# NVlabs/FasterViT

Measured on AMD Instinct MI355X. Metric: images/sec FasterViT-0 224x224 inference, bs=256/GPU, higher is better.
Workload: dtype f16; 1 GPU; faster_vit_0_224 inference, 224x224, batch 256/GPU, synthetic weights (tests/synth.py init family); global_batch=256, parallelism=dp1 (independent shards, no data-path collective), hat_operands=f16, streams=1

## Files before the change

fastervit_amd/csrc/fvit_api.hip:

```cpp
#include <stdarg.h>
#include <stdlib.h>
#include <string.h>

#include <algorithm>
#include <map>
#include <mutex>
#include <string>
#include <vector>

#include "fvit_common.h"

namespace fvit {

static thread_local char g_err[512] = "";

void set_error(const char* fmt, ...) {
    va_list ap;
    va_start(ap, fmt);
    vsnprintf(g_err, sizeof(g_err), fmt, ap);
    va_end(ap);
}

int check_launch(const char* what) {
    hipError_t e = hipGetLastError();
// ... 120 lines not shown
    L.off_SLAB = L.off_CNT = 0;
    if (d.C == 512 && winmlp_supported(d.C, d.hidden)) {
        L.off_SLAB = take(winmlp_split_slab_bytes(L.Mx, d.C, 4));
        L.off_CNT = take((size_t)(L.Mx / 32 + 8) * 4);
    }
    L.off_SPLITK = 0;
    L.splitk_bytes = 0;
    if (tune_get("gemm_splitk", 0)) {
        const int slots = tune_get("gemm_splitk_slots", 460);
        auto need = [&](int64_t rows) -> size_t {
            if (rows <= 0) return 0;
            const int64_t tiles = ((rows + 127) / 128) * ((d.C + 127) / 128);
            const int64_t sp = std::min<int64_t>(8, slots / std::max<int64_t>(tiles, 1));
            return sp >= 2 ? (size_t)sp * rows * d.C * 4 : 0;
        };
        const size_t nb = std::max(need(L.Mx), d.hier ? need(L.Mc) : (size_t)0);
        if (nb > 0) { L.off_SPLITK = take(nb); L.splitk_bytes = nb; }
    }
    L.total = off;
    const int want_s = fvit_attention_spad(L.S), want_g = d.hier ? fvit_attention_spad(L.G) : d.gpad;
    if (d.spad != want_s || d.gpad != want_g) {
        set_error("stage descriptor: spad/gpad %d/%d do not match fvit_attention_spad (%d/%d)", d.spad, d.gpad, want_s, want_g);
        return false;
    }
    return true;
}

#define FVIT_TRY(expr)            \
    do {                          \
        int rc__ = (expr);        \
        if (rc__ != FVIT_OK) return rc__; \
    } while (0)

static AttnBlkCall attnblk_call(int dtype, const float* srcA, int rowsA, const float* srcB, int rowsB, const int32_t* src_idx,
                                const int32_t* add_idx, const float* add, const float* ln_w, const float* ln_b, float eps, int rows_per_image,
                                const void* w_qkv_frag, const float* b_qkv_heads, const void* w_proj_frag, const float* b_proj,
                                const float* gamma, const float* bias, float* x_out, int nwin, int S, int heads, int C, float scale) {
    return {dtype, srcA, rowsA, srcB, rowsB, src_idx, add_idx, add, ln_w, ln_b, eps, rows_per_image, w_qkv_frag,
            b_qkv_heads, w_proj_frag, b_proj, gamma, bias, x_out, nwin, S, heads, C, scale};
}

static MlpFusedCall mlp_fused_call(int dtype, float* x, int M, int C, int hidden, const float* ln_w, const float* ln_b, float eps,
                                   const void* w_fc1_frag, const float* b_fc1, const void* w_fc2_frag, const float* b_fc2, const float* gamma) {
    return {dtype, x, M, C, hidden, ln_w, ln_b, eps, w_fc1_frag, b_fc1, w_fc2_frag, b_fc2, gamma};
}

static CtBlkCall ctblk_call(int dtype, const float* X, int rowsA, const int32_t* src_idx, const float* add, float* R, int batch, int G,
                            int heads, int C, int hidden, const float* ln1_w, const float* ln1_b, const void* w_qkv_frag,
                            const float* b_qkv_heads, const void* w_proj_frag, const float* b_proj, const float* gamma1, const float* bias,
                            float scale, const float* ln2_w, const float* ln2_b, const void* w_fc1_frag, const float* b_fc1,
                            const void* w_fc2_frag, const float* b_fc2, const float* gamma2, float eps) {
    return {dtype, X, rowsA, src_idx, add, R, batch, G, heads, C, hidden, ln1_w, ln1_b, w_qkv_frag, b_qkv_heads, w_proj_frag,
            b_proj, gamma1, bias, scale, ln2_w, ln2_b, w_fc1_frag, b_fc1, w_fc2_frag, b_fc2, gamma2, eps};
}

enum class CarrierRoute {
    NONE,
    FUSED_CT,
    ATTNBLK,
    LNGEMM_CHAIN,
    CHAIN,
};
enum class WinAttnRoute {
    WINBLK,
    ATTNBLK,
    LNGEMM_PREADDED,
    CHAIN,
};
enum class MlpRoute {
    WINMLP,
    MLP_FUSED,
    LNGEMM_CHAIN,
    CHAIN,
};

struct BlockRoute {
    CarrierRoute carrier = CarrierRoute::NONE;
    MlpRoute carrier_mlp = MlpRoute::CHAIN;
    WinAttnRoute window_attn = WinAttnRoute::CHAIN;
    MlpRoute window_mlp = MlpRoute::CHAIN;
    bool preadd_eligible = false;
    const float* pe_next = nullptr;
    int win_blk_split = 1, win_mlp_split = 1;
};

struct RouteKnobs {
    const int ln_gemm = tune_get("ln_gemm", 0), ln_gemm_max_rows = tune_get("ln_gemm_max_rows", 16384);
    const int attn_fused = tune_get("attn_fused", 1), attn_fused_x2 = tune_get("attn_fused_x2", 1);
    const int attn_fused_min_rows = tune_get("attn_fused_min_rows", 16384), attn_fused512_min_rows = tune_get("attn_fused512_min_rows", 1 << 30);
    const int mlp_fused = tune_get("mlp_fused", 1);
    const int mlp_fused_min_rows = tune_get("mlp_fused_min_rows", 16384), mlp_fused512_min_rows = tune_get("mlp_fused512_min_rows", 1 << 30);
    const int win_mlp = tune_get("win_mlp", 1), win_mlp256 = tune_get("win_mlp256", 2), win_mlp_split = tune_get("win_mlp_split", 1);
    const int win_fused = tune_get("win_fused", 1), win_fused256 = tune_get("win_fused256", 0), win_blk_split = tune_get("win_blk_split", 1);
    const int ct_fused = tune_get("ct_fused", 1), pe_preadd = tune_get("pe_preadd", 1);
};

static BlockRoute choose_route(const FvitStageDesc& d, const StageLayout& L, const FvitBlockWeights& w, const RouteKnobs& k) {
    const int T = d.weight_terms;
    auto ln_gemm_ok = [&](int N, int ldo, int64_t rows) {
        return T == 1 && ln_gemm_supported(d.C, N, L.ldn, ldo) && k.ln_gemm && rows <= k.ln_gemm_max_rows;
    };
    auto attnblk = [&](const FvitAttnWeights& a, int S, int64_t rows) {
        const bool terms_ok = T == 1 || (T == 2 && d.C == 256 && S > 48 && k.attn_fused_x2);
        return terms_ok && a.w_qkv_frag && a.b_qkv_heads && a.w_proj_frag && d.dpad == 32 && d.C / d.heads == 32 && attnblk_supported(d.C, d.heads, S) &&
               rows >= (d.C == 256 ? k.attn_fused_min_rows : k.attn_fused512_min_rows) && k.attn_fused;
    };
    auto mlp = [&](const FvitMlpWeights& m, int64_t rows) {
        const bool frags = m.w_fc1_frag && m.w_fc2_frag;
        if (T <= 2 && frags && winmlp_supported(d.C, d.hidden) && (d.C == 512 ? k.win_mlp != 0 : rows >= k.mlp_fused_min_rows && k.win_mlp256 != 0))
            return MlpRoute::WINMLP;
        if (T == 1 && frags && mlp_fused_supported(d.C, d.hidden) && rows >= (d.C == 256 ? k.mlp_fused_min_rows : k.mlp_fused512_min_rows) && k.mlp_fused)
            return MlpRoute::MLP_FUSED;
        return ln_gemm_ok(d.hidden, L.ldh, rows) ? MlpRoute::LNGEMM_CHAIN : MlpRoute::CHAIN;
    };

    BlockRoute r;
    r.win_blk_split = k.win_blk_split;
    r.win_mlp_split = k.win_mlp_split;
    if (d.hier) {
        const FvitAttnWeights& a = w.hat_attn;
        if (T <= 2 && ctblk_supported(d.C, d.heads, L.G, d.hidden) && d.dpad == 32 && a.w_qkv_frag && a.b_qkv_heads && a.w_proj_frag && a.bias &&
            w.hat_mlp.w_fc1_frag && w.hat_mlp.w_fc2_frag && k.ct_fused)
            r.carrier = CarrierRoute::FUSED_CT;
        else if (attnblk(a, L.G, L.Mc))
            r.carrier = CarrierRoute::ATTNBLK;
        else
            r.carrier = ln_gemm_ok(L.ldqkv, L.ldqkv, L.Mc) ? CarrierRoute::LNGEMM_CHAIN : CarrierRoute::CHAIN;
        r.carrier_mlp = mlp(w.hat_mlp, L.Mc);
    }
    const FvitAttnWeights& a = w.attn;
    if (T <= 2 && (T == 1 || d.C == 512) && winblk_supported(d.C, d.heads, L.S) && d.dpad == 32 && a.w_qkv_frag && a.b_qkv_heads && a.w_proj_frag && a.bias &&
        (d.C == 512 ? k.win_fused != 0 : k.win_fused256 != 0))
        r.window_attn = WinAttnRoute::WINBLK;
    else if (attnblk(a, L.S, L.Mx))
        r.window_attn = WinAttnRoute::ATTNBLK;
    r.window_mlp = mlp(w.mlp, L.Mx);
    r.preadd_eligible = !d.hier && r.window_attn == WinAttnRoute::CHAIN && (r.window_mlp == MlpRoute::CHAIN || r.window_mlp == MlpRoute::LNGEMM_CHAIN) &&
                        ln_gemm_ok(L.ldqkv, L.ldqkv, L.Mx) && k.pe_preadd;
    return r;
}

struct Branch {
    float* x;
    int64_t rows;
    void *xn, *qkv, *ao, *h;
    int nwin, S;
};

static LnCall ln_call(const FvitStageDesc& d, const StageLayout& L, const float* ln_w, const float* ln_b, const float* src, int64_t rows, void* n_out) {
    LnCall ln = {d.operand_dtype, src, 0, nullptr, 0, nullptr, nullptr, nullptr, nullptr, n_out, L.at * L.ldn, ln_w, ln_b, 1e-5f, (int)rows, 1, d.C};
    if (L.at == 2) ln.lo_off = L.ldn;
    return ln;
}

enum class AttnStart { QKV_GEMM, CORE };

static int run_attn(const FvitStageDesc& d, const StageLayout& L, const FvitAttnWeights& w, AttnStart start, const Branch& b, char* ws, hipStream_t st) {
    const int dt = d.operand_dtype;
    const int T = d.weight_terms;
    const int AT = L.at;
    dbg_rowhash("attn.xn", b.xn, b.rows, AT * L.ldn * 2, st);
    if (start == AttnStart::QKV_GEMM) {
        GemmCall g1 = {dt, b.xn, AT * L.ldn, w.w_qkv, T * L.ldn, w.b_qkv, nullptr, b.qkv, AT * L.ldqkv, (int)b.rows, L.ldqkv, T * L.ldn, 0};
        g1.ka = L.ldn;
        if (AT == 2) g1.out_lo_off = L.ldqkv;
        FVIT_TRY(launch_gemm(g1, st));
    }
    dbg_rowhash("attn.qkv", b.qkv, b.rows, AT * L.ldqkv * 2, st);
    AttnCall at = {dt, b.qkv, AT * L.ldqkv, b.ao, AT * L.ldao, w.bias, b.nwin, b.S, d.heads, d.dpad, L.scale, w.rel_table, w.rel_w, w.rel_ng, d.C / d.heads};
    if (AT == 2) { at.q_lo_off = L.ldqkv; at.o_lo_off = L.ldao; }
    FVIT_TRY(launch_attention(at, st));
    dbg_rowhash("attn.ao", b.ao, b.rows, AT * L.ldao * 2, st);
    GemmCall g2 = {dt, b.ao, AT * L.ldao, w.w_proj, T * L.ldao, w.b_proj, w.gamma, b.x, d.C, (int)b.rows, d.C, T * L.ldao, 2};
    g2.ka = L.ldao;
    if (L.splitk_bytes) { g2.splitk_slab = (float*)(ws + L.off_SPLITK); g2.splitk_bytes = L.splitk_bytes; }
    FVIT_TRY(launch_gemm(g2, st));
    dbg_rowhash("attn.out", b.x, b.rows, d.C * 4, st);
    return FVIT_OK;
}

static int run_mlp(const FvitStageDesc& d, const StageLayout& L, const FvitMlpWeights& w, MlpRoute route, const BlockRoute& r, const Branch& b,
                   const FvitStageTables& t, char* ws, hipStream_t st) {
    const int dt = d.operand_dtype;
    const int T = d.weight_terms, AT = L.at;
    switch (route) {
    case MlpRoute::WINMLP: {
        MlpFusedCall mc = mlp_fused_call(dt, b.x, (int)b.rows, d.C, d.hidden, w.ln_w, w.ln_b, 1e-5f, w.w_fc1_frag, w.b_fc1, w.w_fc2_frag, w.b_fc2, w.gamma);
        mc.terms = T;
        if (L.off_SLAB) {
            mc.slab = (float*)(ws + L.off_SLAB);
            mc.counters = (int*)(ws + L.off_CNT);
            mc.nsplit = r.win_mlp_split;
        }
        FVIT_TRY(launch_winmlp(mc, st));
        dbg_rowhash("winmlp.out", b.x, b.rows, d.C * 4, st);
        return FVIT_OK;
    }
    case MlpRoute::MLP_FUSED: {
        MlpFusedCall mc = mlp_fused_call(dt, b.x, (int)b.rows, d.C, d.hidden, w.ln_w, w.ln_b, 1e-5f, w.w_fc1_frag, w.b_fc1, w.w_fc2_frag, w.b_fc2, w.gamma);
        dbg_rowhash("mlpf.in", b.x, b.rows, d.C * 4, st);
        FVIT_TRY(launch_mlp_fused(mc, st));
        dbg_rowhash("mlpf.out", b.x, b.rows, d.C * 4, st);
        return FVIT_OK;
    }
    case MlpRoute::LNGEMM_CHAIN: {
        LnGemmCall lg = {ln_call(d, L, w.ln_w, w.ln_b, b.x, b.rows, b.xn), w.w_fc1, L.ldn, w.b_fc1, b.h, L.ldh, d.hidden, 1};
        FVIT_TRY(launch_ln_gemm(lg, st));
        break;
    }
    case MlpRoute::CHAIN: {
        FVIT_TRY(launch_gather_layernorm(ln_call(d, L, w.ln_w, w.ln_b, b.x, b.rows, b.xn), st));
        GemmCall g1 = {dt, b.xn, AT * L.ldn, w.w_fc1, T * L.ldn, w.b_fc1, nullptr, b.h, AT * L.ldh, (int)b.rows, d.hidden, T * L.ldn, 1};
        g1.ka = L.ldn;
        if (AT == 2) g1.out_lo_off = L.ldh;
        FVIT_TRY(launch_gemm(g1, st));
        break;
    }
    }
    dbg_rowhash("mlp.h", b.h, b.rows, AT * L.ldh * 2, st);
    GemmCall g2 = {dt, b.h, AT * L.ldh, w.w_fc2, T * L.ldh, w.b_fc2, w.gamma, b.x, d.C, (int)b.rows, d.C, T * L.ldh, 2};
    g2.ka = L.ldh;
    if (r.pe_next) { g2.add = r.pe_next; g2.add_idx = t.ln1_add; g2.rows_per_image = L.rpi; }
    if (L.splitk_bytes) { g2.splitk_slab = (float*)(ws + L.off_SPLITK); g2.splitk_bytes = L.splitk_bytes; }
    FVIT_TRY(launch_gemm(g2, st));
    dbg_rowhash("mlp.out", b.x, b.rows, d.C * 4, st);
    return FVIT_OK;
}

static AttnBlkCall window_attnblk_call(const FvitStageDesc& d, const StageLayout& L, const FvitBlockWeights& w, const FvitStageTables& t, float* X, float* R) {
    const FvitAttnWeights& a = w.attn;
    AttnBlkCall ab = attnblk_call(d.operand_dtype, X, L.rpi, R, L.G, (d.hier ? t.ln1_src : nullptr), t.ln1_add, w.pe_x, a.ln_w, a.ln_b, 1e-5f, L.rpi,
                                  a.w_qkv_frag, a.b_qkv_heads, a.w_proj_frag, a.b_proj, a.gamma, a.bias, X, d.batch * L.nW, L.S, d.heads, d.C, L.scale);
    ab.terms = d.weight_terms;
    return ab;
}

static int run_block(const FvitStageDesc& d, const StageLayout& L, const BlockRoute& r, const FvitBlockWeights& w, const FvitStageTables& t,
                     char* ws, hipStream_t st) {
    const int dt = d.operand_dtype;
    float* X = (float*)(ws + L.off_X);
    float* R = (float*)(ws + L.off_R);
    const Branch win = {X, L.Mx, ws + L.off_Xn, ws + L.off_QKV, ws + L.off_AO, ws + L.off_H, d.batch * L.nW, L.S};
    const Branch ct = {R, L.Mc, ws + L.off_Rn, ws + L.off_RQKV, ws + L.off_RAO, ws + L.off_RH, d.batch, L.G};

    const FvitAttnWeights& ha = w.hat_attn;
    const float* pe_ct = d.square ? w.pe_ct : nullptr;
    LnCall ct_ln = ln_call(d, L, ha.ln_w, ha.ln_b, X, L.Mc, ct.xn);
    ct_ln.rowsA = L.rpi; ct_ln.src_idx = t.ct_src; ct_ln.add = pe_ct; ct_ln.x_out = R; ct_ln.rows_per_image = L.G;
    switch (r.carrier) {
    case CarrierRoute::NONE:
        break;
    case CarrierRoute::FUSED_CT: {
        const FvitMlpWeights& hm = w.hat_mlp;
        CtBlkCall cb = ctblk_call(dt, X, L.rpi, t.ct_src, pe_ct, R, d.batch, L.G, d.heads, d.C, d.hidden, ha.ln_w, ha.ln_b, ha.w_qkv_frag,
                                  ha.b_qkv_heads, ha.w_proj_frag, ha.b_proj, ha.gamma, ha.bias, L.scale, hm.ln_w, hm.ln_b, hm.w_fc1_frag, hm.b_fc1,
                                  hm.w_fc2_frag, hm.b_fc2, hm.gamma, 1e-5f);
        cb.terms = d.weight_terms;
        FVIT_TRY(launch_ctblk(cb, st));
        dbg_rowhash("ct.block", R, L.Mc, d.C * 4, st);
        break;
    }
    case CarrierRoute::ATTNBLK: {
        AttnBlkCall ab = attnblk_call(dt, X, L.rpi, nullptr, 0, t.ct_src, nullptr, pe_ct, ha.ln_w, ha.ln_b, 1e-5f, L.G, ha.w_qkv_frag, ha.b_qkv_heads,
                                      ha.w_proj_frag, ha.b_proj, ha.gamma, ha.bias, R, d.batch, L.G, d.heads, d.C, L.scale);
        FVIT_TRY(launch_attnblk(ab, st));
        dbg_rowhash("ct.attnblk", R, L.Mc, d.C * 4, st);
        break;
    }
    case CarrierRoute::LNGEMM_CHAIN: {
        LnGemmCall lg = {ct_ln, ha.w_qkv, L.ldn, ha.b_qkv, ct.qkv, L.ldqkv, L.ldqkv, 0};
        FVIT_TRY(launch_ln_gemm(lg, st));
        FVIT_TRY(run_attn(d, L, ha, AttnStart::CORE, ct, ws, st));
        break;
    }
    case CarrierRoute::CHAIN:
        FVIT_TRY(launch_gather_layernorm(ct_ln, st));
        dbg_rowhash("ct.gather", R, L.Mc, d.C * 4, st);
        FVIT_TRY(run_attn(d, L, ha, AttnStart::QKV_GEMM, ct, ws, st));
        break;
    }
    if (r.carrier != CarrierRoute::NONE && r.carrier != CarrierRoute::FUSED_CT) FVIT_TRY(run_mlp(d, L, w.hat_mlp, r.carrier_mlp, r, ct, t, ws, st));

    const FvitAttnWeights& a = w.attn;
    switch (r.window_attn) {
    case WinAttnRoute::WINBLK: {
        AttnBlkCall ab = window_attnblk_call(d, L, w, t, X, R);
        if (L.off_SLAB) {
            ab.slab = (float*)(ws + L.off_SLAB);
            ab.counters = (int*)(ws + L.off_CNT);
            ab.nsplit = r.win_blk_split;
        }
        FVIT_TRY(launch_winblk(ab, st));
        dbg_rowhash("win.winblk", X, L.Mx, d.C * 4, st);
        break;
    }
    case WinAttnRoute::ATTNBLK:
        FVIT_TRY(launch_attnblk(window_attnblk_call(d, L, w, t, X, R), st));
        dbg_rowhash("win.attnblk", X, L.Mx, d.C * 4, st);
        break;
    case WinAttnRoute::LNGEMM_PREADDED: {
        LnGemmCall lg = {ln_call(d, L, a.ln_w, a.ln_b, X, L.Mx, nullptr), a.w_qkv, L.ldn, a.b_qkv, win.qkv, L.ldqkv, L.ldqkv, 0};
        FVIT_TRY(launch_ln_gemm(lg, st));
        FVIT_TRY(run_attn(d, L, a, AttnStart::CORE, win, ws, st));
        break;
    }
    case WinAttnRoute::CHAIN: {
        LnCall ln1 = ln_call(d, L, a.ln_w, a.ln_b, X, L.Mx, win.xn);
        ln1.rowsA = L.rpi; ln1.srcB = R; ln1.rowsB = L.G; ln1.src_idx = d.hier ? t.ln1_src : nullptr; ln1.add_idx = t.ln1_add; ln1.add = w.pe_x;
        ln1.x_out = X; ln1.rows_per_image = L.rpi;
        FVIT_TRY(launch_gather_layernorm(ln1, st));
        dbg_rowhash("win.gather", X, L.Mx, d.C * 4, st);
        FVIT_TRY(run_attn(d, L, a, AttnStart::QKV_GEMM, win, ws, st));
        break;
    }
    }
    return run_mlp(d, L, w.mlp, r.window_mlp, r, win, t, ws, st);
}

static int check_hat_call(const FvitStageDesc* desc, bool args_ok, const FvitStageTables* t, const void* workspace, size_t workspace_bytes,
                          const void* carrier, const char* no_carrier, StageLayout& L) {
    if (!desc || !args_ok) {
        set_error("null argument");
        return FVIT_EINVAL;
    }
    const FvitStageDesc& d = *desc;
    if (!make_layout(d, L)) return FVIT_EINVAL;
    if (!t || !t->ln1_add || (d.hier && (!t->ln1_src || !t->ct_src)) || (d.hier && d.do_propagation && !t->up_idx)) {
        set_error("stage tables missing (ln1_add%s)", d.hier ? ", ln1_src, ct_src, up_idx" : "");
        return FVIT_EINVAL;
    }
    if (!workspace || workspace_bytes < L.total) {
        set_error("workspace too small: %zu < %zu", workspace_bytes, L.total);
        return FVIT_EWORKSPACE;
    }
    if (d.hier && !carrier) {
        set_error("%s", no_carrier);
        return FVIT_EINVAL;
    }
    return FVIT_OK;
}

}

using namespace fvit;

extern "C" {

int fvit_abi_version(void) { return FVIT_ABI_VERSION; }
const char* fvit_last_error(void) { return g_err; }

int fvit_attention_dense(int32_t S, int32_t dpad) { return attention_dense(S, dpad) ? 1 : 0; }

int fvit_attention_spad(int32_t S) {
    int sb = (S + 15) / 16;
    if (sb == 9) sb = 10;
    if (sb == 11 || sb == 12) sb = 13;
    return sb * 16;
}

size_t fvit_stage_workspace_bytes(const FvitStageDesc* desc) {
    StageLayout L;
    if (!desc || !make_layout(*desc, L)) return 0;
    return L.total;
}

int fvit_workspace_init(const FvitStageDesc* desc, void* workspace, size_t bytes, fvit_stream_t stream) {
    StageLayout L;
    if (!desc || !make_layout(*desc, L)) return FVIT_EINVAL;
    if (!workspace || bytes < L.total) {
        set_error("workspace too small: %zu < %zu", bytes, L.total);
        return FVIT_EWORKSPACE;
    }
    if (hipMemsetAsync(workspace, 0, L.total, (hipStream_t)stream) != hipSuccess) return check_launch("workspace memset");
    return FVIT_OK;
}

int fvit_hat_stage_forward(const FvitStageDesc* desc, const FvitBlockWeights* blocks, const FvitStageTables* tables,
                           const FvitMapView* in, const float* ct_init, const FvitMapView* out, void* workspace,
                           size_t workspace_bytes, fvit_stream_t stream) {
    return fvit_hat_stage_forward_tail(desc, blocks, tables, in, ct_init, out, nullptr, workspace, workspace_bytes, stream);
}

int fvit_rows_avgpool(int32_t round_dtype, const float* x, float* out, int32_t B, int32_t rows, int32_t C, fvit_stream_t stream) {
    return launch_rows_avgpool(x, out, B, rows, C, round_dtype, (hipStream_t)stream);
}

int fvit_hat_stage_forward_tail(const FvitStageDesc* desc, const FvitBlockWeights* blocks, const FvitStageTables* tables,
                                const FvitMapView* in, const float* ct_init, const FvitMapView* out, const FvitStageTail* tail,
                                void* workspace, size_t workspace_bytes, fvit_stream_t stream) {
    StageLayout L;
    const bool pooled = tail && tail->pool_out;
    FVIT_TRY(check_hat_call(desc, blocks && in && (out || pooled), tables, workspace, workspace_bytes, ct_init, "hierarchical stage needs ct_init", L));
    const FvitStageDesc& d = *desc;
    if (tail && (!tail->ln_w != !tail->ln_b || (pooled && tail->ln_w))) {
        set_error("stage tail: LayerNorm2d needs both ln_w and ln_b, and excludes pool_out");
        return FVIT_EINVAL;
    }
    if (pooled && (d.hier || L.nW != 1 || L.ncw != 0 || d.H != d.Hp || d.W != d.Wp)) {
        set_error("stage tail: pool_out needs one window per image and no carrier tokens (hier=%d, %d windows, map %dx%d of %dx%d)", d.hier, L.nW, d.H, d.W,
                  d.Hp, d.Wp);
        return FVIT_EINVAL;
    }
    hipStream_t st = (hipStream_t)stream;
    char* ws = (char*)workspace;
    float* X = (float*)(ws + L.off_X);
    PartitionCall pc = {*in, d.batch, d.C, d.Hp, d.Wp, d.ws, X, L.S, L.ncw, d.hier ? ct_init : nullptr, L.ncw};
    FVIT_TRY(launch_partition(pc, st));
    dbg_rowhash("partition", X, L.Mx, d.C * 4, st);
    const RouteKnobs knobs{};
    std::vector<BlockRoute> routes;
    for (int i = 0; i < d.depth; ++i) routes.push_back(choose_route(d, L, blocks[i], knobs));
    for (int i = 0; i + 1 < d.depth; ++i) {
        if (routes[i].preadd_eligible && routes[i + 1].preadd_eligible && blocks[i + 1].pe_x) {
            routes[i].pe_next = blocks[i + 1].pe_x;
            routes[i + 1].window_attn = WinAttnRoute::LNGEMM_PREADDED;
        }
    }
    for (int i = 0; i < d.depth; ++i) FVIT_TRY(run_block(d, L, routes[i], blocks[i], *tables, ws, st));
    if (pooled)
        return launch_rows_avgpool(X, tail->pool_out, d.batch, L.S, d.C, tail->pool_dtype, st);
    const bool prop = d.hier && d.do_propagation && d.depth > 0 && blocks[d.depth - 1].last;
    ReverseCall rc = {X, L.S, L.ncw, d.batch, d.C, d.Hp, d.Wp, d.H, d.W, d.ws, *out,
                      prop ? blocks[d.depth - 1].hat_attn.gamma : nullptr, prop ? tables->up_idx : nullptr};
    if (tail && tail->ln_w) return launch_reverse_ln(rc, tail->ln_w, tail->ln_b, tail->ln_eps, st);
    FVIT_TRY(launch_reverse(rc, st));
    return FVIT_OK;
}

int fvit_hat_block_forward(const FvitStageDesc* desc, const FvitBlockWeights* block, const FvitStageTables* tables, float* x,
                           float* ct, void* workspace, size_t workspace_bytes, fvit_stream_t stream) {
    StageLayout L;
    FVIT_TRY(check_hat_call(desc, block && x, tables, workspace, workspace_bytes, ct, "hierarchical block needs carrier tokens", L));
    const FvitStageDesc& d = *desc;
    hipStream_t st = (hipStream_t)stream;
    char* ws = (char*)workspace;
    float* X = (float*)(ws + L.off_X);
    const int nwin = d.batch * L.nW;
    FVIT_TRY(launch_ct_copy(X, L.S, L.ncw, L.nloc, x, nwin, d.C, 1, st));
    if (d.hier) FVIT_TRY(launch_ct_copy(X, L.S, 0, L.ncw, ct, nwin, d.C, 1, st));
    FVIT_TRY(run_block(d, L, choose_route(d, L, *block, RouteKnobs{}), *block, *tables, ws, st));
    if (d.hier && block->last && d.do_propagation)
        FVIT_TRY(launch_propagate(X, block->hat_attn.gamma, tables->up_idx, L.S, L.ncw, L.nloc, nwin, d.C, st));
    FVIT_TRY(launch_ct_copy(X, L.S, L.ncw, L.nloc, x, nwin, d.C, 0, st));
    if (d.hier) FVIT_TRY(launch_ct_copy(X, L.S, 0, L.ncw, ct, nwin, d.C, 0, st));
    return FVIT_OK;
}

int fvit_token_init(const FvitMapView* in, const float* weight, const float* bias, float* ct_out, int32_t batch, int32_t C, int32_t Hp,
                    int32_t Wp, int32_t pool_kh, int32_t pool_kw, int32_t pool_sh, int32_t pool_sw, int32_t cw, fvit_stream_t stream) {
    if (!in || !weight || !bias || !ct_out) { set_error("null argument"); return FVIT_EINVAL; }
    return launch_token_init(*in, weight, bias, ct_out, batch, C, Hp, Wp, pool_kh, pool_kw, pool_sh, pool_sw, cw, (hipStream_t)stream);
}

int fvit_window_partition(const FvitMapView* in, int32_t batch, int32_t C, int32_t Hp, int32_t Wp, int32_t ws, float* windows,
                          fvit_stream_t stream) {
    if (!in || !windows) { set_error("null argument"); return FVIT_EINVAL; }
    PartitionCall pc = {*in, batch, C, Hp, Wp, ws, windows, ws * ws, 0, nullptr, 0};
    return launch_partition(pc, (hipStream_t)stream);
}

int fvit_window_reverse(const float* windows, int32_t batch, int32_t C, int32_t Hp, int32_t Wp, int32_t H, int32_t W, int32_t ws,
                        const FvitMapView* out, fvit_stream_t stream) {
    if (!out || !windows) { set_error("null argument"); return FVIT_EINVAL; }
    ReverseCall rc = {windows, ws * ws, 0, batch, C, Hp, Wp, H, W, ws, *out, nullptr, nullptr};
    return launch_reverse(rc, (hipStream_t)stream);
}

int fvit_gemm_bias_act(int32_t operand_dtype, const void* A, int32_t lda, const void* Wt, int32_t ldw, const float* bias, void* out,
                       int32_t ldo, int32_t M, int32_t N, int32_t K, int32_t act, fvit_stream_t stream) {
    GemmCall g = {operand_dtype, A, lda, Wt, ldw, bias, nullptr, out, ldo, M, N, K, act ? 1 : 0};
    return launch_gemm(g, (hipStream_t)stream);
}

int fvit_gemm_residual(int32_t operand_dtype, const void* A, int32_t lda, const void* Wt, int32_t ldw, const float* bias,
                       const float* gamma, float* x, int32_t ldx, int32_t M, int32_t N, int32_t K, fvit_stream_t stream) {
    GemmCall g = {operand_dtype, A, lda, Wt, ldw, bias, gamma, x, ldx, M, N, K, 2};
    return launch_gemm(g, (hipStream_t)stream);
}

int fvit_gemm_residual_splitk(int32_t operand_dtype, const void* A, int32_t lda, const void* Wt, int32_t ldw, const float* bias, const float* gamma,
                              float* x, int32_t ldx, int32_t M, int32_t N, int32_t K, float* slab, size_t slab_bytes, fvit_stream_t stream) {
    GemmCall g = {operand_dtype, A, lda, Wt, ldw, bias, gamma, x, ldx, M, N, K, 2};
    g.splitk_slab = slab;
    g.splitk_bytes = slab_bytes;
    return launch_gemm(g, (hipStream_t)stream);
}

int fvit_gemm_terms(int32_t operand_dtype, const void* A, int32_t lda, const void* Wt, int32_t ldw, const float* bias, const float* gamma,
                    void* out, int32_t ldo, int32_t M, int32_t N, int32_t K, int32_t ka, int32_t epilogue, fvit_stream_t stream) {
    if (epilogue < 0 || epilogue > 2) { set_error("gemm_terms: epilogue %d", epilogue); return FVIT_EINVAL; }
    GemmCall g = {operand_dtype, A, lda, Wt, ldw, bias, epilogue == 2 ? gamma : nullptr, out, ldo, M, N, K, epilogue};
    g.ka = ka;
    return launch_gemm(g, (hipStream_t)stream);
}

int fvit_gemm_terms_lo(int32_t operand_dtype, const void* A, int32_t lda, const void* Wt, int32_t ldw, const float* bias, const float* gamma,
                       void* out, int32_t ldo, int32_t out_lo_off, int32_t M, int32_t N, int32_t K, int32_t ka, int32_t epilogue,
                       fvit_stream_t stream) {
    if (epilogue < 0 || epilogue > 2) { set_error("gemm_terms_lo: epilogue %d", epilogue); return FVIT_EINVAL; }
    GemmCall g = {operand_dtype, A, lda, Wt, ldw, bias, epilogue == 2 ? gamma : nullptr, out, ldo, M, N, K, epilogue};
    g.ka = ka;
    g.out_lo_off = out_lo_off;
    return launch_gemm(g, (hipStream_t)stream);
}

int fvit_window_attention_terms(int32_t operand_dtype, const void* qkv, int32_t ldq, int32_t q_lo_off, void* out, int32_t ldo,
// ... 310 lines not shown
```

fastervit_amd/csrc/fvit_attnblk.hip:

```cpp
#include "fvit_common.h"

namespace fvit {

namespace {

struct AttnBlkParams {
    const float* srcA;
    const float* srcB;
    const int32_t* src_idx;
    const int32_t* add_idx;
    const float* add;
    const float* ln_w;
    const float* ln_b;
    float eps;
    int rowsA, rowsB, rows_per_image;
    const void* wqkv_f;
    const float* bqkv;
    const void* wproj_f;
    const float* bproj;
    const float* gamma;
    const float* bias;
    float* x_out;
    int nwin, S, heads;
    float scale;
    int ablate;
    unsigned long long* ts;
    int stagger;
};

__device__ __forceinline__ void glds16(const void* gsrc, char* lds_dst) {
    __builtin_amdgcn_global_load_lds((const __attribute__((address_space(1))) void*)gsrc,
                                     (__attribute__((address_space(3))) void*)lds_dst, 16, 0, 0);
}

template <typename T, int CC, int NRB, int NW, bool BIAS_LDS, bool DBQ = false, bool TS = false, int WT = 1>
__global__ __launch_bounds__(64 * NW, (CC == 256 && WT == 1) ? 2 : 1) void attnblk_kernel(AttnBlkParams p) {
    static_assert(WT == 1 || (WT == 2 && DBQ && !BIAS_LDS && !TS), "two weight terms: DBQ form, bias from L2");
    typedef typename Op16<T>::v8 v8;
#define FVIT_AB_STAMP(k) if constexpr (TS) { if ((threadIdx.x & 63) == 0) p.ts[((size_t)blockIdx.x * NW + (threadIdx.x >> 6)) * 16 + (k)] = __builtin_amdgcn_s_memtime(); }
    FVIT_AB_STAMP(0)
    typedef typename Op16<T>::v4 v4;
    constexpr int C = CC, KK = C / 32, CB = C / 16;
    constexpr int SP = NRB * 16;
    constexpr int WPW = NW / NRB;
    constexpr int NKB32 = (NRB + 1) / 2;
    constexpr int QKV_FRAGS = 6 * KK;
    constexpr int QKV_BYTES = QKV_FRAGS * 1024, PROJ_BYTES = CB * 1024, BIAS_BYTES = BIAS_LDS ? SP * SP * 4 : 0;
    constexpr int KX_BYTES = NW * 1024;
    constexpr int VX_BYTES = WPW * 2 * NKB32 * 1024;
    constexpr int OFF_PROJ = (DBQ ? 2 : 1) * QKV_BYTES, OFF_BIAS = OFF_PROJ + WT * PROJ_BYTES, OFF_KX = OFF_BIAS + ((BIAS_BYTES + 1023) / 1024) * 1024;
    constexpr int OFF_VX = OFF_KX + KX_BYTES, OFF_BQ = OFF_VX + VX_BYTES;
    constexpr int MAX_HEADS = CC / 32;
    constexpr int OFF_BP = OFF_BQ + MAX_HEADS * 96 * 4;
    __shared__ __attribute__((aligned(16))) char smem[OFF_BP + 2 * CC * 4];

    const int tid = threadIdx.x;
    const int lane = tid & 63;
    const int wave = __builtin_amdgcn_readfirstlane(tid >> 6);
    const int g = lane >> 4, s = lane & 15;
    const int lane16 = lane * 16;
    const int wi = wave / NRB, qb = wave - wi * NRB;
    const int win = blockIdx.x * WPW + wi;
    const bool win_ok = win < p.nwin;
    const int tok = qb * 16 + s;
    const bool row_ok = win_ok && tok < p.S;
    const int64_t row = (int64_t)(win_ok ? win : p.nwin - 1) * p.S + (tok < p.S ? tok : p.S - 1);
    float* bqs = (float*)(smem + OFF_BQ);
    float* bps = (float*)(smem + OFF_BP);
    float* gms = bps + CC;

    const char* __restrict__ Wq = (const char*)p.wqkv_f;
    const char* __restrict__ Wp = (const char*)p.wproj_f;

    auto dma_qkv = [&](int h, int slot, int term = 0) {
        const char* src = Wq + ((size_t)term * p.heads + h) * QKV_BYTES + lane16;
        char* dst = smem + slot * QKV_BYTES;
#pragma unroll
        for (int i = 0; i < QKV_FRAGS / NW; ++i) glds16(src + (wave + NW * i) * 1024, dst + (wave + NW * i) * 1024);
    };
    auto dma_proj_bias = [&](int h) {
        const char* src = Wp + (size_t)h * PROJ_BYTES + lane16;
#pragma unroll
        for (int i = 0; i < CB / NW; ++i) glds16(src + (wave + NW * i) * 1024, smem + OFF_PROJ + (wave + NW * i) * 1024);
        if constexpr (WT == 2) {
            const char* src2 = Wp + ((size_t)p.heads + h) * PROJ_BYTES + lane16;
#pragma unroll
            for (int i = 0; i < CB / NW; ++i) glds16(src2 + (wave + NW * i) * 1024, smem + OFF_PROJ + PROJ_BYTES + (wave + NW * i) * 1024);
        }
        if (BIAS_LDS) {
            const char* bsrc = (const char*)(p.bias + (size_t)h * SP * SP) + lane16;
            constexpr int BP = (BIAS_BYTES + 1023) / 1024;
#pragma unroll
            for (int i = 0; i < (BP + NW - 1) / NW; ++i) {
                const int piece = wave + NW * i;
                if (piece < BP) glds16(bsrc + piece * 1024, smem + OFF_BIAS + piece * 1024);
            }
        }
    };

    for (int i = tid; i < p.heads * 96; i += 64 * NW) bqs[i] = p.bqkv[i];
    for (int i = tid; i < CC; i += 64 * NW) {
        bps[i] = p.bproj[i];
        gms[i] = p.gamma ? p.gamma[i] : 1.0f;
    }
    if (NRB == 1) {
        for (int i = tid; i < VX_BYTES / 4; i += 64 * NW) ((float*)(smem + OFF_VX))[i] = 0.f;
    }
    const int hrot = p.stagger ? (int)((blockIdx.x >> 3) % (unsigned)p.heads) : 0;
    auto head_of = [&](int it) { const int hh = it + hrot; return hh >= p.heads ? hh - p.heads : hh; };
    dma_qkv(head_of(0), 0);
    if constexpr (WT == 2) dma_qkv(head_of(0), 1, 1);

    const float* src;
    const float* addp = nullptr;
    {
        const int b = (int)(row / p.rows_per_image), pr = (int)(row - (int64_t)b * p.rows_per_image);
        if (p.src_idx) {
            const int si = p.src_idx[pr];
            src = si >= 0 ? p.srcA + ((size_t)b * p.rowsA + si) * C : p.srcB + ((size_t)b * p.rowsB + (-si - 1)) * C;
        } else {
            src = p.srcA + (size_t)row * C;
        }
        if (p.add) {
            const int ai = p.add_idx ? p.add_idx[pr] : pr;
            if (ai >= 0) addp = p.add + (size_t)ai * C;
        }
    }
    constexpr bool KEEPX = CC == 256;
    v8 xf[KK];
    f4 v[KK][2];
    {
        float sum = 0.f;
#pragma unroll
        for (int kk = 0; kk < KK; ++kk)
#pragma unroll
            for (int h2 = 0; h2 < 2; ++h2) {
                const int co = (kk >> 1) * 64 + g * 16 + (kk & 1) * 8 + h2 * 4;
                f4 t = *(const f4*)(src + co);
                if (addp) t += *(const f4*)(addp + co);
                v[kk][h2] = t;
                sum += (t[0] + t[1]) + (t[2] + t[3]);
            }
        sum = sum_xor32(sum_xor16(sum));
        if constexpr (TS) { asm volatile("s_nop 0" ::"v"(sum) : "memory"); }
        FVIT_AB_STAMP(1)
        const float mean = sum / (float)C;
        float sq = 0.f;
#pragma unroll
        for (int kk = 0; kk < KK; ++kk)
#pragma unroll
            for (int h2 = 0; h2 < 2; ++h2) {
                const f4 d = v[kk][h2] - mean;
                sq += (d[0] * d[0] + d[1] * d[1]) + (d[2] * d[2] + d[3] * d[3]);
            }
        sq = sum_xor32(sum_xor16(sq));
        const float rstd = rsqrtf(sq / (float)C + p.eps);
#pragma unroll
        for (int kk = 0; kk < KK; ++kk) {
            v8 o;
#pragma unroll
            for (int h2 = 0; h2 < 2; ++h2) {
                const int co = (kk >> 1) * 64 + g * 16 + (kk & 1) * 8 + h2 * 4;
                const f4 w = *(const f4*)(p.ln_w + co);
                const f4 b = *(const f4*)(p.ln_b + co);
#pragma unroll
                for (int r = 0; r < 4; ++r) o[h2 * 4 + r] = sat16<T>((v[kk][h2][r] - mean) * rstd * w[r] + b[r]);
            }
            xf[kk] = o;
        }
    }

    f4 oacc[CB];
#pragma unroll
    for (int cb = 0; cb < CB; ++cb) oacc[cb] = (f4){0.f, 0.f, 0.f, 0.f};
    if constexpr (TS) { asm volatile("s_nop 0" ::"v"(xf[KK - 1]) : "memory"); }
    FVIT_AB_STAMP(2)

    const char* wq_base = smem + lane16;
    const char* wp_l = smem + OFF_PROJ + lane16;
    const float* bias_l = (const float*)(smem + OFF_BIAS);
    char* kx = smem + OFF_KX;
    char* vx = smem + OFF_VX;

    for (int hit = 0; hit < p.heads; ++hit) {
        const int h = head_of(hit);
        asm volatile("s_waitcnt vmcnt(0)" ::: "memory");
        __syncthreads();
        f4 bzg[NRB];
        if (!BIAS_LDS) {
            const float* bg = p.bias + ((size_t)h * SP + tok) * SP + g * 4;
#pragma unroll
            for (int kb = 0; kb < NRB; ++kb) bzg[kb] = *(const f4*)(bg + kb * 16);
        }
        if (!(p.ablate & 1)) dma_proj_bias(h);
        const bool next_q = DBQ && hit + 1 < p.heads && !(p.ablate & 1);
        if constexpr (WT == 1) {
            if (next_q) dma_qkv(head_of(hit + 1), (hit + 1) & 1);
        }
        const char* wq_l = wq_base + ((DBQ && WT == 1) ? (hit & 1) * QKV_BYTES : 0);

        f4 acc[6];
#pragma unroll
        for (int ub = 0; ub < 6; ++ub) acc[ub] = (f4){0.f, 0.f, 0.f, 0.f};
#pragma unroll
        for (int term = 0; term < WT; ++term) {
            if (WT == 2 && term == 1) {
                asm volatile("s_waitcnt lgkmcnt(0)\n\ts_barrier" ::: "memory");
                if (next_q) dma_qkv(head_of(hit + 1), 0, 0);
                wq_l = wq_base + QKV_BYTES;
            }
            v8 wa[6], wb[6];
#pragma unroll
            for (int ub = 0; ub < 6; ++ub) wa[ub] = *(const v8*)(wq_l + (ub * KK + 0) * 1024);
#pragma unroll
            for (int kk = 0; kk < KK; kk += 2) {
                __builtin_amdgcn_sched_barrier(0);
#pragma unroll
                for (int ub = 0; ub < 6; ++ub) wb[ub] = *(const v8*)(wq_l + (ub * KK + kk + 1) * 1024);
                __builtin_amdgcn_sched_barrier(0);
#pragma unroll
                for (int ub = 0; ub < 4; ++ub) acc[ub] = Op16<T>::mfma(wa[ub], xf[kk], acc[ub]);
// ... 46 lines not shown
        }

        f4 sc[NRB];
        float mx = -3.0e38f;
#pragma unroll
        for (int kb = 0; kb < NRB; ++kb) {
            const v8 kfa = *(const v8*)(kx + (wi * NRB + kb) * 1024 + lane16);
            f4 a = Op16<T>::mfma(kfa, qf, (f4){0.f, 0.f, 0.f, 0.f});
            const f4 bz = BIAS_LDS ? *(const f4*)(bias_l + tok * SP + kb * 16 + g * 4) : bzg[kb];
#pragma unroll
            for (int r = 0; r < 4; ++r) {
                a[r] = a[r] * p.scale + bz[r];
                mx = fmaxf(mx, a[r]);
            }
            sc[kb] = a;
        }
        mx = max_xor32(max_xor16(mx));
        float sum = 0.f;
#pragma unroll
        for (int kb = 0; kb < NRB; ++kb)
#pragma unroll
            for (int r = 0; r < 4; ++r) {
                const float e = __expf(sc[kb][r] - mx);
                sc[kb][r] = e;
                sum += e;
            }
        sum = sum_xor32(sum_xor16(sum));
        const float inv = 1.0f / sum;
        f4 o[2] = {(f4){0.f, 0.f, 0.f, 0.f}, (f4){0.f, 0.f, 0.f, 0.f}};
#pragma unroll
        for (int k32 = 0; k32 < NKB32; ++k32) {
            v8 pf;
#pragma unroll
            for (int r = 0; r < 4; ++r) {
                pf[r] = (T)sc[2 * k32][r];
                pf[4 + r] = (2 * k32 + 1 < NRB) ? (T)sc[(2 * k32 + 1 < NRB) ? 2 * k32 + 1 : 0][r] : (T)0.f;
            }
#pragma unroll
            for (int db = 0; db < 2; ++db) {
                const v8 vf = *(const v8*)(vx + ((wi * 2 + db) * NKB32 + k32) * 1024 + lane16);
                o[db] = Op16<T>::mfma(vf, pf, o[db]);
            }
        }
        v8 of;
#pragma unroll
        for (int r = 0; r < 4; ++r) {
            of[r] = sat16<T>(o[0][r] * inv);
            of[4 + r] = sat16<T>(o[1][r] * inv);
        }
#pragma unroll
        for (int term = 0; term < WT; ++term) {
            constexpr int PB = 4;
            const char* wp_t = wp_l + term * PROJ_BYTES;
            v8 pa[PB], pb[PB];
#pragma unroll
            for (int i = 0; i < PB; ++i) pa[i] = *(const v8*)(wp_t + i * 1024);
#pragma unroll
            for (int c0 = 0; c0 < CB; c0 += 2 * PB) {
                __builtin_amdgcn_sched_barrier(0);
#pragma unroll
                for (int i = 0; i < PB; ++i) pb[i] = *(const v8*)(wp_t + (c0 + PB + i) * 1024);
                __builtin_amdgcn_sched_barrier(0);
#pragma unroll
                for (int i = 0; i < PB; ++i) oacc[c0 + i] = Op16<T>::mfma(pa[i], of, oacc[c0 + i]);
                __builtin_amdgcn_sched_barrier(0);
                if (c0 + 2 * PB < CB) {
#pragma unroll
                    for (int i = 0; i < PB; ++i) pa[i] = *(const v8*)(wp_t + (c0 + 2 * PB + i) * 1024);
                    __builtin_amdgcn_sched_barrier(0);
                }
#pragma unroll
                for (int i = 0; i < PB; ++i) oacc[c0 + PB + i] = Op16<T>::mfma(pb[i], of, oacc[c0 + PB + i]);
            }
        }
        if constexpr (TS) {
            asm volatile("s_nop 0" ::"v"(oacc[CB - 1]) : "memory");
            if (hit < 8) { FVIT_AB_STAMP(3 + hit) }
        }
    }
    FVIT_AB_STAMP(14)

    if (row_ok) {
        float* px = p.x_out + (size_t)row * C;
#pragma unroll
        for (int cg = 0; cg < CB / 4; ++cg) {
            const int c0 = cg * 64 + g * 16;
#pragma unroll
            for (int q = 0; q < 4; ++q) {
                f4 xv;
                if (KEEPX) {
                    xv = v[2 * cg + (q >> 1)][q & 1];
                } else {
                    xv = *(const f4*)(src + c0 + q * 4);
                    if (addp) xv += *(const f4*)(addp + c0 + q * 4);
                }
                const f4 bv = *(const f4*)(bps + c0 + q * 4);
                const f4 gv = *(const f4*)(gms + c0 + q * 4);
                const f4 a = oacc[cg * 4 + q];
#pragma unroll
                for (int r = 0; r < 4; ++r) xv[r] += gv[r] * (a[r] + bv[r]);
                *(f4*)(px + c0 + q * 4) = xv;
            }
        }
    }
    if constexpr (TS) { asm volatile("s_waitcnt vmcnt(0)" ::: "memory"); }
    FVIT_AB_STAMP(15)
#undef FVIT_AB_STAMP
}

}

bool attnblk_supported(int C, int heads, int S) {
    if (C == 256 && heads == 8) return (S >= 1 && S <= 16) || (S > 48 && S <= 64);
    return C == 512 && heads == 16 && S > 48 && S <= 64;
}

int launch_attnblk(const AttnBlkCall& c, hipStream_t stream) {
    if (ablate_skip(8)) return FVIT_OK;
    if (!attnblk_supported(c.C, c.heads, c.S) || c.nwin <= 0 || !c.wqkv_f || !c.wproj_f || !c.x_out) {
        set_error("attn_block: unsupported arguments C=%d heads=%d S=%d nwin=%d", c.C, c.heads, c.S, c.nwin);
        return FVIT_EINVAL;
    }
    AttnBlkParams p;
    p.srcA = c.srcA; p.srcB = c.srcB; p.src_idx = c.src_idx; p.add_idx = c.add_idx; p.add = c.add; p.ln_w = c.ln_w; p.ln_b = c.ln_b;
    p.eps = c.eps; p.rowsA = c.rowsA; p.rowsB = c.rowsB; p.rows_per_image = c.rows_per_image > 0 ? c.rows_per_image : 1;
    p.wqkv_f = c.wqkv_f; p.bqkv = c.bqkv; p.wproj_f = c.wproj_f; p.bproj = c.bproj; p.gamma = c.gamma; p.bias = c.bias;
    p.x_out = c.x_out; p.nwin = c.nwin; p.S = c.S; p.heads = c.heads; p.scale = c.scale;
    p.ablate = diag_knob("ab_ablate");
    p.stagger = tune_get("ab_stagger", 0);
    p.ts = (unsigned long long*)c.ts;
    const double rows = (double)c.nwin * c.S;
    const double flops = 2.0 * rows * c.C * 4.0 * c.C + 4.0 * c.nwin * (double)c.heads * c.S * (double)c.S * 32.0;
    const double bytes = 8.0 * rows * c.C + 8.0 * c.C * c.C;
    ProfScope prof(FVIT_K_ATTN_FUSED, flops, bytes, stream);
    prof_note(c.C == 256 ? (c.S <= 16 ? "attnblk_kernel<256,S16>" : "attnblk_kernel<256,S64>") : "attnblk_kernel<512,S64>", c.nwin);
    const bool small = c.S <= 16;
    if (attnblk2_supported(c.C, c.heads, c.S) && c.terms == 1 && tune_get("ab_variant", 0) == 3) return launch_attnblk2(c, stream);
    if (c.terms != 1 && (c.terms != 2 || c.C != 256 || small)) {
        set_error("attn_block: weight terms %d at C=%d S=%d (two terms: C = 256, 48 < S <= 64 only)", c.terms, c.C, c.S);
        return FVIT_EINVAL;
    }
    if (c.terms == 2) {
        prof_note("attnblk_kernel<256,S64,2 terms>", (c.nwin + 1) / 2);
        if (c.ts) { set_error("attn_block timeline: one weight term only"); return FVIT_EINVAL; }
        if (c.dtype == FVIT_F16) hipLaunchKernelGGL((attnblk_kernel<_Float16, 256, 4, 8, false, true, false, 2>), dim3((c.nwin + 1) / 2), dim3(512), 0, stream, p);
        else if (c.dtype == FVIT_BF16) hipLaunchKernelGGL((attnblk_kernel<__bf16, 256, 4, 8, false, true, false, 2>), dim3((c.nwin + 1) / 2), dim3(512), 0, stream, p);
        else { set_error("attn_block: operand dtype %d not supported", c.dtype); return FVIT_EINVAL; }
        return check_launch("attnblk_kernel");
    }
    const int variant = tune_get("ab_variant", 0);
#define FVIT_AB(T, NRB, NW, BL) do { \
        if (c.C == 256) hipLaunchKernelGGL((attnblk_kernel<T, 256, NRB, NW, BL>), dim3((c.nwin + (NW / NRB) - 1) / (NW / NRB)), dim3(64 * NW), 0, stream, p); \
        else hipLaunchKernelGGL((attnblk_kernel<T, 512, 4, 4, false>), dim3(c.nwin), dim3(256), 0, stream, p); \
    } while (0)
#define FVIT_AB_DBQ(T) hipLaunchKernelGGL((attnblk_kernel<T, 256, 4, 8, true, true>), dim3((c.nwin + 1) / 2), dim3(512), 0, stream, p)
    const bool dbq = variant == 2 && c.C == 256 && !small;
    if (c.ts) {
        if (c.dtype != FVIT_F16 || c.C != 256 || small) { set_error("attn_block timeline: fp16, C = 256, 48 < S <= 64 only"); return FVIT_EINVAL; }
        hipLaunchKernelGGL((attnblk_kernel<_Float16, 256, 4, 4, false, false, true>), dim3(c.nwin), dim3(256), 0, stream, p);
        return check_launch("attnblk_kernel");
    }
    if (c.dtype == FVIT_F16) {
        if (small) FVIT_AB(_Float16, 1, 8, true);
        else if (dbq) FVIT_AB_DBQ(_Float16);
        else if (variant == 1) FVIT_AB(_Float16, 4, 8, true);
        else FVIT_AB(_Float16, 4, 4, false);
    } else if (c.dtype == FVIT_BF16) {
        if (small) FVIT_AB(__bf16, 1, 8, true);
        else if (dbq) FVIT_AB_DBQ(__bf16);
        else if (variant == 1) FVIT_AB(__bf16, 4, 8, true);
        else FVIT_AB(__bf16, 4, 4, false);
    } else {
        set_error("attn_block: operand dtype %d not supported", c.dtype);
        return FVIT_EINVAL;
    }
#undef FVIT_AB
#undef FVIT_AB_DBQ
    return check_launch("attnblk_kernel");
}

}
```

fastervit_amd/csrc/fvit_common.h:

```cpp
#pragma once
#include <hip/hip_runtime.h>
#include <stdint.h>
#include <atomic>
#include <mutex>
#include <stdio.h>

#include "../../include/fvit_hip.h"

namespace fvit {

typedef _Float16 h8 __attribute__((ext_vector_type(8)));
typedef _Float16 h4 __attribute__((ext_vector_type(4)));
typedef __bf16 b8 __attribute__((ext_vector_type(8)));
typedef __bf16 b4 __attribute__((ext_vector_type(4)));
typedef float f4 __attribute__((ext_vector_type(4)));

template <typename T> struct Op16;
template <> struct Op16<_Float16> {
    typedef h8 v8;
    typedef h4 v4;
    static __device__ __forceinline__ f4 mfma(v8 a, v8 b, f4 c) {
        return __builtin_amdgcn_mfma_f32_16x16x32_f16(a, b, c, 0, 0, 0);
    }
};
template <> struct Op16<__bf16> {
    typedef b8 v8;
    typedef b4 v4;
    static __device__ __forceinline__ f4 mfma(v8 a, v8 b, f4 c) {
        return __builtin_amdgcn_mfma_f32_16x16x32_bf16(a, b, c, 0, 0, 0);
    }
};

template <typename T> __device__ __forceinline__ T sat16(float x);
template <> __device__ __forceinline__ _Float16 sat16<_Float16>(float x) { return (_Float16)__builtin_amdgcn_fmed3f(x, -65504.0f, 65504.0f); }
template <> __device__ __forceinline__ __bf16 sat16<__bf16>(float x) { return (__bf16)x; }

__device__ __forceinline__ float sum_xor16(float x) {
    const auto r = __builtin_amdgcn_permlane16_swap(__float_as_uint(x), __float_as_uint(x), false, false);
    return __uint_as_float(r[0]) + __uint_as_float(r[1]);
}
__device__ __forceinline__ float sum_xor32(float x) {
    const auto r = __builtin_amdgcn_permlane32_swap(__float_as_uint(x), __float_as_uint(x), false, false);
    return __uint_as_float(r[0]) + __uint_as_float(r[1]);
}
__device__ __forceinline__ float max_xor16(float x) {
    const auto r = __builtin_amdgcn_permlane16_swap(__float_as_uint(x), __float_as_uint(x), false, false);
    return fmaxf(__uint_as_float(r[0]), __uint_as_float(r[1]));
}
__device__ __forceinline__ float max_xor32(float x) {
    const auto r = __builtin_amdgcn_permlane32_swap(__float_as_uint(x), __float_as_uint(x), false, false);
    return fmaxf(__uint_as_float(r[0]), __uint_as_float(r[1]));
}

template <int CTRL>
__device__ __forceinline__ float dpp_lane(float x) {
    return __int_as_float(__builtin_amdgcn_update_dpp(0, __float_as_int(x), CTRL, 0xf, 0xf, false));
}
template <int N>
__device__ __forceinline__ float group_sum(float x) {
    static_assert(N >= 1 && N <= 64 && (N & (N - 1)) == 0, "group size");
    if constexpr (N >= 2) x += dpp_lane<0xB1>(x);
    if constexpr (N >= 4) x += dpp_lane<0x4E>(x);
    if constexpr (N >= 8) x += dpp_lane<0x141>(x);
    if constexpr (N >= 16) x += dpp_lane<0x140>(x);
    if constexpr (N >= 32) x = sum_xor16(x);
    if constexpr (N >= 64) x = sum_xor32(x);
    return x;
}
template <int N>
__device__ __forceinline__ float group_max(float x) {
    static_assert(N >= 1 && N <= 64 && (N & (N - 1)) == 0, "group size");
    if constexpr (N >= 2) x = fmaxf(x, dpp_lane<0xB1>(x));
    if constexpr (N >= 4) x = fmaxf(x, dpp_lane<0x4E>(x));
    if constexpr (N >= 8) x = fmaxf(x, dpp_lane<0x141>(x));
    if constexpr (N >= 16) x = fmaxf(x, dpp_lane<0x140>(x));
    if constexpr (N >= 32) x = max_xor16(x);
    if constexpr (N >= 64) x = max_xor32(x);
    return x;
}

__device__ __forceinline__ float fast_erf(float x) {
    const float ax = fabsf(x);
    const float t = __frcp_rn(1.0f + 0.3275911f * ax);
    float y = 1.061405429f;
    y = y * t - 1.453152027f;
    y = y * t + 1.421413741f;
    y = y * t - 0.284496736f;
    y = y * t + 0.254829592f;
    y = 1.0f - y * t * __expf(-ax * ax);
    return copysignf(y, x);
}
__device__ __forceinline__ float gelu_fast(float x) {
    const float z = __builtin_amdgcn_fmed3f(x * 0.70710678118654752f, -3.0f, 3.0f);
    const float u = z * z;
    float q = 4.075095461e-08f;
    q = q * u - 1.945139275e-06f;
    q = q * u + 4.106515917e-05f;
    q = q * u - 5.110726343e-04f;
    q = q * u + 4.235583358e-03f;
    q = q * u - 2.510324307e-02f;
    q = q * u + 1.110798195e-01f;
    q = q * u - 3.753151596e-01f;
    q = q * u + 1.128268480e+00f;
    const float hx = 0.5f * x;
    return hx * (z * q) + hx;
}

template <int N>
__device__ __forceinline__ void pin_values(float (&q)[N]) {
    static_assert(N == 4 || N == 8, "pin_values: 4 or 8 values");
    if constexpr (N == 4) asm("" : "+v"(q[0]), "+v"(q[1]), "+v"(q[2]), "+v"(q[3]));
    else asm("" : "+v"(q[0]), "+v"(q[1]), "+v"(q[2]), "+v"(q[3]), "+v"(q[4]), "+v"(q[5]), "+v"(q[6]), "+v"(q[7]));
}
template <int N>
__device__ __forceinline__ void gelu_fast_n(float (&x)[N]) {
    float z[N], u[N], q[N];
#pragma unroll
    for (int i = 0; i < N; ++i) z[i] = __builtin_amdgcn_fmed3f(x[i] * 0.70710678118654752f, -3.0f, 3.0f);
#pragma unroll
    for (int i = 0; i < N; ++i) u[i] = z[i] * z[i];
    pin_values(u);
#pragma unroll
    for (int i = 0; i < N; ++i) q[i] = 4.075095461e-08f * u[i] - 1.945139275e-06f;
#define FVIT_GELU_STEP(c) \
    pin_values(q);        \
    _Pragma("unroll") for (int i = 0; i < N; ++i) q[i] = q[i] * u[i] + (c);
    FVIT_GELU_STEP(4.106515917e-05f)
    FVIT_GELU_STEP(-5.110726343e-04f)
    FVIT_GELU_STEP(4.235583358e-03f)
    FVIT_GELU_STEP(-2.510324307e-02f)
    FVIT_GELU_STEP(1.110798195e-01f)
    FVIT_GELU_STEP(-3.753151596e-01f)
    FVIT_GELU_STEP(1.128268480e+00f)
#undef FVIT_GELU_STEP
    pin_values(q);
#pragma unroll
    for (int i = 0; i < N; ++i) {
        const float hx = 0.5f * x[i];
        x[i] = hx * (z[i] * q[i]) + hx;
    }
}

template <int M>
__device__ __forceinline__ void gelu_fast_each(float (&x)[M]) {
    static_assert(M % 4 == 0, "gelu_fast_each: a multiple of 4 values");
#pragma unroll
    for (int j = 0; j + 8 <= M; j += 8) {
        float t[8];
#pragma unroll
        for (int i = 0; i < 8; ++i) t[i] = x[j + i];
        gelu_fast_n<8>(t);
#pragma unroll
        for (int i = 0; i < 8; ++i) x[j + i] = t[i];
    }
    if constexpr (M % 8 == 4) {
        float t[4];
#pragma unroll
        for (int i = 0; i < 4; ++i) t[i] = x[M - 4 + i];
        gelu_fast_n<4>(t);
#pragma unroll
        for (int i = 0; i < 4; ++i) x[M - 4 + i] = t[i];
// ... 52 lines not shown
}

__host__ __device__ constexpr int round_up(int x, int m) { return (x + m - 1) / m * m; }
static inline int64_t round_up64(int64_t x, int64_t m) { return (x + m - 1) / m * m; }

struct DeviceOnce {
    std::atomic<uint64_t> mask{0};
    bool first_on_current_device() {
        int dev = 0;
        if (hipGetDevice(&dev) != hipSuccess || dev < 0 || dev > 63) return true;
        const uint64_t bit = 1ull << dev;
        return (mask.fetch_or(bit) & bit) == 0;
    }
};

void set_error(const char* fmt, ...);
int check_launch(const char* what);

int tune_get(const char* key, int dflt);
#ifdef FVIT_DIAG
inline bool ablate_skip(int bit) { return (tune_get("ablate_skip", 0) & bit) != 0; }
inline int diag_knob(const char* key) { return tune_get(key, 0); }
#else
inline bool ablate_skip(int) { return false; }
inline int diag_knob(const char*) { return 0; }
#endif

std::recursive_mutex& diag_mutex();

struct ProfScope {
    ProfScope(int kind, double flops, double bytes, hipStream_t stream);
    ~ProfScope();
    int slot_;
    hipStream_t stream_;
};
void prof_note(const char* kernel, int grid);
#ifdef FVIT_DIAG
void dbg_poison_before_launch(hipStream_t st);
void dbg_rowhash(const char* tag, const void* ptr, long long rows, int row_bytes, hipStream_t st);
#else
inline void dbg_poison_before_launch(hipStream_t) {}
inline void dbg_rowhash(const char*, const void*, long long, int, hipStream_t) {}
#endif

struct GemmCall {
    int dtype;
    const void* A;
    int lda;
    const void* W;
    int ldw;
    const float* bias;
    const float* gamma;
    void* out;
    int ldo;
    int M, N, K;
    int epilogue;
    const float* add = nullptr;
    const int32_t* add_idx = nullptr;
    int rows_per_image = 1;
    int ka = 0;
    int out_lo_off = 0;
    float* splitk_slab = nullptr;
    size_t splitk_bytes = 0;
};
int launch_gemm(const GemmCall& c, hipStream_t stream);

struct MlpFusedCall {
    int dtype;
    float* x;
    int M, C, hidden;
    const float* ln_w;
    const float* ln_b;
    float eps;
    const void* w1f;
    const float* b1;
    const void* w2f;
    const float* b2;
    const float* gamma;
    int terms = 1;
    float* slab = nullptr;
    int* counters = nullptr;
    int nsplit = 1;
    void* ts = nullptr;
};
size_t winmlp_split_slab_bytes(int64_t M, int C, int nsplit);
bool mlp_fused_supported(int C, int hidden);
int launch_mlp_fused(const MlpFusedCall& c, hipStream_t stream);
bool winmlp_supported(int C, int hidden);
int launch_winmlp(const MlpFusedCall& c, hipStream_t stream);

struct AttnBlkCall {
    int dtype;
    const float* srcA;
    int rowsA;
    const float* srcB;
    int rowsB;
    const int32_t* src_idx;
    const int32_t* add_idx;
    const float* add;
    const float* ln_w;
    const float* ln_b;
    float eps;
    int rows_per_image;
    const void* wqkv_f;
    const float* bqkv;
    const void* wproj_f;
    const float* bproj;
    const float* gamma;
    const float* bias;
    float* x_out;
    int nwin, S, heads, C;
    float scale;
    float* slab = nullptr;
    int* counters = nullptr;
    int nsplit = 1;
    int terms = 1;
    void* ts = nullptr;
};
bool attnblk_supported(int C, int heads, int S);
int launch_attnblk(const AttnBlkCall& c, hipStream_t stream);
bool attnblk2_supported(int C, int heads, int S);
int launch_attnblk2(const AttnBlkCall& c, hipStream_t stream);
bool winblk_supported(int C, int heads, int S);
int launch_winblk(const AttnBlkCall& c, hipStream_t stream);
struct AttnCall {
    int dtype;
    const void* qkv;
    int ldq;
    void* out;
    int ldo;
    const float* bias;
    int nwin, S, heads, dpad;
    float scale;
    const float* rel_table;
    int rel_w, rel_ng;
    int d;
    int q_lo_off = 0, o_lo_off = 0;
    const void* drop_mask = nullptr;
};
bool attention_dense(int S, int dpad);
int launch_attention(const AttnCall& c, hipStream_t stream);
int launch_attention_long(const AttnCall& c, hipStream_t stream);

struct LnCall {
    int dtype;
    const float* srcA;
    int rowsA;
    const float* srcB;
    int rowsB;
    const int32_t* src_idx;
    const int32_t* add_idx;
    const float* add;
    float* x_out;
    void* n_out;
    int ldn;
    const float* ln_w;
    const float* ln_b;
    float eps;
    int rows, rows_per_image, C;
    int lo_off = 0;
};
int launch_gather_layernorm(const LnCall& c, hipStream_t stream);

struct CtBlkCall {
    int dtype;
    const float* X; int rowsA;
    const int32_t* src_idx;
    const float* add;
    float* R;
    int batch, G, heads, C, hidden;
    const float* ln1_w; const float* ln1_b; const void* wqkv_f; const float* bqkv; const void* wproj_f; const float* bproj; const float* gamma1;
    const float* bias; float scale;
    const float* ln2_w; const float* ln2_b; const void* w1f; const float* b1; const void* w2f; const float* b2; const float* gamma2;
    float eps;
    int terms = 1;
    void* ts = nullptr;
};
bool ctblk_supported(int C, int heads, int G, int hidden);
int launch_ctblk(const CtBlkCall& c, hipStream_t stream);

struct LnGemmCall {
    LnCall ln;
    const void* W;
    int ldw;
    const float* bias;
    void* out;
    int ldo;
    int N;
    int epilogue;
};
bool ln_gemm_supported(int C, int N, int ldw, int ldo);
int launch_ln_gemm(const LnGemmCall& c, hipStream_t stream);

struct PartitionCall {
    FvitMapView in;
    int batch, C, Hp, Wp, ws;
    float* x;
    int rows_per_win;
    int row_off;
    const float* ct;
    int ncw;
};
int launch_partition(const PartitionCall& c, hipStream_t stream);

struct ReverseCall {
    const float* x;
    int rows_per_win, row_off;
    int batch, C, Hp, Wp, H, W, ws;
    FvitMapView out;
    const float* gamma;
    const int32_t* up_idx;
};
int launch_reverse(const ReverseCall& c, hipStream_t stream);
bool reverse_ln_supported(const ReverseCall& c);
int launch_reverse_ln(const ReverseCall& c, const float* ln_w, const float* ln_b, float eps, hipStream_t stream);
int launch_rows_avgpool(const float* x, float* out, int batch, int rows, int C, int round_dtype, hipStream_t stream);

int launch_ct_copy(float* x, int rows_per_win, int row_off, int ncw, float* ct, int nwin_total, int C, int to_x,
                   hipStream_t stream);
int launch_token_init(const FvitMapView& in, const float* w, const float* bias, float* out, int B, int C, int Hp, int Wp, int kh, int kw,
                      int sh, int sw, int cw, hipStream_t stream);
int launch_propagate(float* x, const float* gamma, const int32_t* up_idx, int rows_per_win, int ncw, int nloc,
                     int nwin_total, int C, hipStream_t stream);

}
```

fastervit_amd/csrc/fvit_ctblk.hip:

```cpp
#include "fvit_common.h"

namespace fvit {

namespace {

struct CtBlkParams {
    const float* X;
    const int32_t* src_idx;
    const float* add;
    float* R;
    int rowsA, B, G;
    const float* ln1_w; const float* ln1_b;
    const void* wqkv_f;
    const float* bqkv;
    const void* wproj_f;
    const float* bproj; const float* gamma1;
    const float* bias;
    float scale;
    const float* ln2_w; const float* ln2_b;
    const void* w1f;
    const float* b1;
    const void* w2f;
    const float* b2; const float* gamma2;
    float eps;
    int touch;
    unsigned long long* ts;
};

template <typename T, int DEPTH, int MINB, int WT = 1>
__global__ __launch_bounds__(256, MINB) void ctblk_kernel(CtBlkParams p) {
    typedef typename Op16<T>::v8 v8;
    typedef typename Op16<T>::v4 v4;
    constexpr int C = 256, KK = 8, CB = 16, NW = 4, HID = 1024;
    constexpr int CPW = HID / 32 / NW;
    constexpr int SA = 16 * WT;
    constexpr int NSTEP = SA + 4 * WT * CPW;
    constexpr size_t QKV_IMG = (size_t)3 * C * C * 2, PROJ_IMG = (size_t)C * C * 2, FC_IMG = (size_t)C * HID * 2;
    constexpr int OFF_B1 = NW * CB * 1024, OFF_BQ = OFF_B1 + HID * 4, OFF_BZ = OFF_BQ + 8 * 96 * 4;
    __shared__ __attribute__((aligned(16))) char smem[OFF_BZ + 8 * 256 * 4];
    float* b1s = (float*)(smem + OFF_B1);
    float* bqs = (float*)(smem + OFF_BQ);
    float* bzs = (float*)(smem + OFF_BZ);

    const int tid = threadIdx.x;
    const int lane = tid & 63;
    const int wave = __builtin_amdgcn_readfirstlane(tid >> 6);
    const int g = lane >> 4, s = lane & 15;
    const int lane16 = lane * 16;
    const int img = blockIdx.x;
    const int tok = s < p.G ? s : p.G - 1;
    const bool row_ok = s < p.G;

    const char* Wq = (const char*)p.wqkv_f + lane16;
    const char* Wp = (const char*)p.wproj_f + lane16;
    const char* W1 = (const char*)p.w1f + lane16;
    const char* W2 = (const char*)p.w2f + lane16;
    auto step_ptr = [&](int t) -> const char* {
        if (t < SA) {
            const int h = 2 * wave + t / (8 * WT), r = t % (8 * WT), u = r / WT, term = r % WT;
            return u < 6 ? Wq + term * QKV_IMG + ((size_t)h * 48 + u * 8) * 1024 : Wp + term * PROJ_IMG + ((size_t)h * 16 + (u - 6) * 8) * 1024;
        }
        const int m = t - SA, j = CPW * wave + m / (4 * WT), r = m % (4 * WT), u = r / WT, term = r % WT;
        return (u < 2 ? W1 : W2) + term * FC_IMG + ((size_t)j * 16 + (u & 1) * 8) * 1024;
    };
    v8 ring[DEPTH][8];
    constexpr bool in_attention = true;
#define FVIT_CT_LOAD(t)                                                                                  \
    if ((t) < NSTEP && !(in_attention && (t) >= SA)) {                                                                                   \
        const char* sp_ = step_ptr(t);                                                                   \
        _Pragma("unroll") for (int i_ = 0; i_ < 8; ++i_) ring[(t) % DEPTH][i_] = *(const v8*)(sp_ + i_ * 1024); \
    }                                                                                                    \
    __builtin_amdgcn_sched_barrier(0);

    if (p.touch) {
        unsigned sink = 0;
        const unsigned* tq = (const unsigned*)((const char*)p.wqkv_f + (size_t)(2 * wave) * 48 * 1024 + lane * 128);
        const unsigned* tp = (const unsigned*)((const char*)p.wproj_f + (size_t)(2 * wave) * 16 * 1024 + lane * 128);
        const unsigned* t1 = (const unsigned*)((const char*)p.w1f + (size_t)(CPW * wave) * 16 * 1024 + lane * 128);
        const unsigned* t2 = (const unsigned*)((const char*)p.w2f + (size_t)(CPW * wave) * 16 * 1024 + lane * 128);
#pragma unroll
        for (int i = 0; i < 12; ++i) sink ^= tq[i * 2048];
#pragma unroll
        for (int i = 0; i < 4; ++i) sink ^= tp[i * 2048];
#pragma unroll
        for (int i = 0; i < 2 * CPW; ++i) sink ^= t1[i * 2048];
#pragma unroll
        for (int i = 0; i < 2 * CPW; ++i) sink ^= t2[i * 2048];
        if (sink == 0x9E3779B1u && p.touch == 12345) p.R[0] = 0.f;
    }
    {
        float c1[HID / 256], c2[3], c3[8];
#pragma unroll
        for (int i = 0; i < HID / 256; ++i) c1[i] = p.b1[tid + 256 * i];
#pragma unroll
        for (int i = 0; i < 3; ++i) c2[i] = p.bqkv[tid + 256 * i];
#pragma unroll
        for (int i = 0; i < 8; ++i) c3[i] = p.bias[tid + 256 * i];
        __builtin_amdgcn_sched_barrier(0);
#pragma unroll
        for (int t = 0; t < DEPTH; ++t) { FVIT_CT_LOAD(t) }
#pragma unroll
        for (int i = 0; i < HID / 256; ++i) b1s[tid + 256 * i] = c1[i];
#pragma unroll
        for (int i = 0; i < 3; ++i) bqs[tid + 256 * i] = c2[i];
#pragma unroll
        for (int i = 0; i < 8; ++i) bzs[tid + 256 * i] = c3[i];
    }

    const float* src = p.X + ((size_t)img * p.rowsA + p.src_idx[tok]) * C + g * 16;
    const bool has_add = p.add != nullptr, has_g1 = p.gamma1 != nullptr, has_g2 = p.gamma2 != nullptr;
    const float* addp = has_add ? p.add + (size_t)tok * C + g * 16 : src;
    auto gather = [&](f4 (&v)[CB]) {
#pragma unroll
        for (int cb = 0; cb < CB; ++cb) v[cb] = *(const f4*)(src + (cb >> 2) * 64 + (cb & 3) * 4);
#pragma unroll
        for (int cb = 0; cb < CB; ++cb) {
            const f4 a = *(const f4*)(addp + (cb >> 2) * 64 + (cb & 3) * 4);
#pragma unroll
            for (int r = 0; r < 4; ++r) v[cb][r] += has_add ? a[r] : 0.f;
        }
    };
    auto layernorm = [&](const f4 (&v)[CB], const float* lw, const float* lb, v8 (&xf)[KK]) {
        float sum = 0.f;
#pragma unroll
        for (int cb = 0; cb < CB; ++cb) sum += (v[cb][0] + v[cb][1]) + (v[cb][2] + v[cb][3]);
        sum = sum_xor32(sum_xor16(sum));
        const float mean = sum / (float)C;
        float sq = 0.f;
#pragma unroll
        for (int cb = 0; cb < CB; ++cb) {
            const f4 d = v[cb] - mean;
            sq += (d[0] * d[0] + d[1] * d[1]) + (d[2] * d[2] + d[3] * d[3]);
        }
        sq = sum_xor32(sum_xor16(sq));
        const float rstd = rsqrtf(sq / (float)C + p.eps);
#pragma unroll
        for (int kk = 0; kk < KK; ++kk) {
            v8 o;
#pragma unroll
            for (int h2 = 0; h2 < 2; ++h2) {
                const int cb = 2 * kk + h2;
                const int co = (cb >> 2) * 64 + g * 16 + (cb & 3) * 4;
                const f4 w = *(const f4*)(lw + co);
                const f4 b = *(const f4*)(lb + co);
#pragma unroll
                for (int r = 0; r < 4; ++r) o[h2 * 4 + r] = sat16<T>((v[cb][r] - mean) * rstd * w[r] + b[r]);
            }
            xf[kk] = o;
        }
    };

    v8 xf[KK];
    {
        f4 v[CB];
        gather(v);
        layernorm(v, p.ln1_w, p.ln1_b, xf);
    }

    __syncthreads();
    f4 oacc[CB];
#pragma unroll
    for (int cb = 0; cb < CB; ++cb) oacc[cb] = (f4){0.f, 0.f, 0.f, 0.f};
#pragma unroll
    for (int hh = 0; hh < 2; ++hh) {
        const int h = 2 * wave + hh;
        const float* bq = bqs + h * 96;
        v8 qf, kf, vf[2];
#pragma unroll
        for (int ub = 0; ub < 6; ++ub) {
            f4 a = (f4){0.f, 0.f, 0.f, 0.f}, ao = (f4){0.f, 0.f, 0.f, 0.f};
#pragma unroll
            for (int term = 0; term < WT; ++term) {
                const int t = (hh * 8 + ub) * WT + term;
#pragma unroll
                for (int kk = 0; kk < KK; kk += 2) {
                    a = ub < 4 ? Op16<T>::mfma(ring[t % DEPTH][kk], xf[kk], a)
                               : Op16<T>::mfma(xf[kk], ring[t % DEPTH][kk], a);
                    ao = ub < 4 ? Op16<T>::mfma(ring[t % DEPTH][kk + 1], xf[kk + 1], ao) : Op16<T>::mfma(xf[kk + 1], ring[t % DEPTH][kk + 1], ao);
                }
                __builtin_amdgcn_sched_barrier(0);
                FVIT_CT_LOAD(t + DEPTH)
            }
            a += ao;
            if (ub < 4) {
                const f4 bb = *(const f4*)(bq + (ub >> 1) * 32 + (ub & 1) * 16 + g * 4);
#pragma unroll
                for (int r = 0; r < 4; ++r) {
                    if (ub < 2) qf[(ub & 1) * 4 + r] = sat16<T>(a[r] + bb[r]);
                    else kf[(ub & 1) * 4 + r] = sat16<T>(a[r] + bb[r]);
                }
            } else {
                const float bv = bq[64 + (ub - 4) * 16 + s];
// ... 111 lines not shown
        float hv[8];
#pragma unroll
        for (int r = 0; r < 4; ++r) {
            hv[r] = a1[0][r] + bA[r];
            hv[4 + r] = a1[1][r] + bB[r];
        }
        gelu_fast_n<8>(hv);
        v8 pf;
#pragma unroll
        for (int r = 0; r < 8; ++r) pf[r] = sat16<T>(hv[r]);
#pragma unroll
        for (int half = 0; half < 2; ++half)
#pragma unroll
            for (int term = 0; term < WT; ++term) {
                const int t = SA + (4 * c + 2 + half) * WT + term;
#pragma unroll
                for (int i = 0; i < 8; ++i) acc2[half * 8 + i] = Op16<T>::mfma(ring[t % DEPTH][i], pf, acc2[half * 8 + i]);
                __builtin_amdgcn_sched_barrier(0);
                FVIT_CT_LOAD(t + DEPTH)
            }
    }
#undef FVIT_CT_LOAD

#pragma unroll
    for (int cb = 0; cb < CB; ++cb) *(f4*)(ex + (wave * CB + cb) * 1024) = acc2[cb];
    __syncthreads();
    if (row_ok) {
        float* pr = p.R + ((size_t)img * p.G + s) * C + wave * 64 + g * 16;
#pragma unroll
        for (int q = 0; q < 4; ++q) {
            const int cbo = (4 * wave + q) * 1024;
            f4 a = *(const f4*)(ex + (0 * CB) * 1024 + cbo);
#pragma unroll
            for (int w = 1; w < NW; ++w) a += *(const f4*)(ex + (w * CB) * 1024 + cbo);
            const int co = wave * 64 + g * 16 + q * 4;
            const f4 bv = *(const f4*)(p.b2 + co);
            const f4 gl = *(const f4*)((has_g2 ? p.gamma2 : p.b2) + co);
            f4 o = r1q[q];
#pragma unroll
            for (int r = 0; r < 4; ++r) o[r] += (has_g2 ? gl[r] : 1.f) * (a[r] + bv[r]);
            *(f4*)(pr + q * 4) = o;
        }
    }
}


template <typename T, int WT, int DEPTH, bool TS = false, int NIMG = 1>
__global__ __launch_bounds__(512, 1) void ctblk8_kernel(CtBlkParams p) {
    typedef typename Op16<T>::v8 v8;
    static_assert(!TS || NIMG == 1, "timeline instance: one image per workgroup");
#define FVIT_CT8_STAMP(k, dep) if constexpr (TS) { asm volatile("s_nop 0" ::"v"(dep) : "memory"); if ((threadIdx.x & 63) == 0) p.ts[((size_t)blockIdx.x * 8 + (threadIdx.x >> 6)) * 16 + (k)] = __builtin_amdgcn_s_memtime(); }
    FVIT_CT8_STAMP(0, threadIdx.x)
    constexpr int C = 256, KK = 8, CB = 16, NW = 8, HID = 1024;
    constexpr int S_QKV = 6 * WT, S_PROJ = 2 * WT, S_FC1 = 8 * WT, S_FC2 = 8 * WT;
    constexpr int T_PROJ = S_QKV, T_FC1 = T_PROJ + S_PROJ, T_FC2 = T_FC1 + S_FC1, NSTEP = T_FC2 + S_FC2;
    constexpr size_t QKV_IMG = (size_t)3 * C * C * 2, PROJ_IMG = (size_t)C * C * 2, FC_IMG = (size_t)C * HID * 2;
    constexpr int OT_B = 8 * 1024, H_B = 32 * 1024, CT_B = CB * 1024;
    constexpr int OFF_B1 = 0, OFF_BQ = OFF_B1 + HID * 4, OFF_BZ = OFF_BQ + 8 * 96 * 4, OFF_VEC = OFF_BZ + 8 * 256 * 4;
    constexpr int OFF_CT = OFF_VEC + 8 * C * 4, OFF_OT = OFF_CT + NIMG * CT_B, OFF_H = OFF_OT + NIMG * OT_B, LDS_BYTES = OFF_H + NIMG * H_B;
    static_assert(OFF_OT <= 65536 && NIMG * OT_B <= 65536 && NIMG * H_B <= 65536, "three bases (constants + ct1 rows, O^T, H^T), 16-bit offsets from each");
    __shared__ __attribute__((aligned(16))) char smem[LDS_BYTES];
    float* b1s = (float*)(smem + OFF_B1);
    float* bqs = (float*)(smem + OFF_BQ);
    float* bzs = (float*)(smem + OFF_BZ);
    float* vecs = (float*)(smem + OFF_VEC);

    const int tid = threadIdx.x;
    const int lane = tid & 63;
    const int wave = __builtin_amdgcn_readfirstlane(tid >> 6);
    const int g = lane >> 4, s = lane & 15;
    const int lane16 = lane * 16;
    char* smH = smem + OFF_H + lane16;
    char* smO = smem + OFF_OT + lane16;
    asm volatile("" : "+v"(smH), "+v"(smO));
    const int img0 = blockIdx.x * NIMG;
    const int tok = s < p.G ? s : p.G - 1;
    const bool row_ok = s < p.G;

    const bool has_add = p.add != nullptr;
    f4 rowq[NIMG][2];
#pragma unroll
    for (int im = 0; im < NIMG; ++im) {
        const int img = min(img0 + im, p.B - 1);
        const float* src = p.X + ((size_t)img * p.rowsA + p.src_idx[tok]) * C + g * 16;
#pragma unroll
        for (int q = 0; q < 2; ++q) {
            const int cb = 2 * wave + q;
            rowq[im][q] = *(const f4*)(src + (cb >> 2) * 64 + (cb & 3) * 4);
        }
    }
    if (has_add) {
        const float* addp = p.add + (size_t)tok * C + g * 16;
#pragma unroll
        for (int q = 0; q < 2; ++q) {
            const int cb = 2 * wave + q;
            const f4 a = *(const f4*)(addp + (cb >> 2) * 64 + (cb & 3) * 4);
#pragma unroll
            for (int im = 0; im < NIMG; ++im) rowq[im][q] += a;
        }
    }
    __builtin_amdgcn_sched_barrier(0);

    const char* Wq = (const char*)p.wqkv_f + lane16;
    const char* Wp = (const char*)p.wproj_f + lane16;
    const char* W1 = (const char*)p.w1f + lane16;
    const char* W2 = (const char*)p.w2f + lane16;
    v8 ring[DEPTH][8];
    auto frag_ptr = [&](int t, int i) -> const char* {
        if (t < T_PROJ) {
            const int ub = t / WT, term = t % WT;
            return Wq + term * QKV_IMG + ((size_t)wave * 48 + ub * 8 + i) * 1024;
        }
        if (t < T_FC1) {
            const int u = t - T_PROJ, half = u / WT, term = u % WT;
            const int h = 4 * half + (i >> 1), cb = 2 * wave + (i & 1);
            return Wp + term * PROJ_IMG + ((size_t)h * CB + cb) * 1024;
        }
        if (t < T_FC2) {
            const int u = t - T_FC1, ch = u / WT, term = u % WT;
            const int j = 4 * wave + (ch >> 1), hb = ch & 1;
            return W1 + term * FC_IMG + ((size_t)j * 16 + hb * 8 + i) * 1024;
        }
        {
            const int u = t - T_FC2, q = u / WT, term = u % WT;
            const int j = 4 * q + (i >> 1), cb = 2 * wave + (i & 1);
            return W2 + term * FC_IMG + ((size_t)j * CB + cb) * 1024;
        }
    };
#define FVIT_CT8_LOAD(t)                                                                                              \
    if ((t) < NSTEP) {                                                                                                \
        _Pragma("unroll") for (int i_ = 0; i_ < 8; ++i_) ring[(t) % DEPTH][i_] = *(const v8*)frag_ptr((t), i_);      \
    }                                                                                                                 \
    __builtin_amdgcn_sched_barrier(0);

    {
        float c1[2], c3[4], c4[4];
        float c2 = 0.f;
#pragma unroll
        for (int i = 0; i < 2; ++i) c1[i] = p.b1[tid + 512 * i];
        if (tid < 8 * 96 - 512) c2 = p.bqkv[tid + 512];
        const float c2a = p.bqkv[tid];
#pragma unroll
        for (int i = 0; i < 4; ++i) c3[i] = p.bias[tid + 512 * i];
        {
            const float* vp[8] = {p.ln1_w, p.ln1_b, p.bproj, p.gamma1, p.ln2_w, p.ln2_b, p.b2, p.gamma2};
            const int hi = tid >> 8, ch = tid & 255;
#pragma unroll
            for (int i = 0; i < 4; ++i) {
                const float* q = hi ? vp[2 * i + 1] : vp[2 * i];
                c4[i] = q ? q[ch] : 1.0f;
            }
        }
        __builtin_amdgcn_sched_barrier(0);
#pragma unroll
        for (int t = 0; t < DEPTH; ++t) { FVIT_CT8_LOAD(t) }
#pragma unroll
        for (int i = 0; i < 2; ++i) b1s[tid + 512 * i] = c1[i];
        bqs[tid] = c2a;
        if (tid < 8 * 96 - 512) bqs[tid + 512] = c2;
#pragma unroll
        for (int i = 0; i < 4; ++i) bzs[tid + 512 * i] = c3[i];
#pragma unroll
        for (int i = 0; i < 4; ++i) vecs[(2 * i + (tid >> 8)) * C + (tid & 255)] = c4[i];
#pragma unroll
        for (int im = 0; im < NIMG; ++im)
#pragma unroll
            for (int q = 0; q < 2; ++q) *(f4*)(smem + OFF_CT + im * CT_B + (2 * wave + q) * 1024 + lane16) = rowq[im][q];
// ... 199 lines not shown
            for (int im = 0; im < NIMG; ++im) a1[im][hb] = a[im] + ao[im];
        }
        const f4 bA = *(const f4*)(b1s + j * 32 + g * 4);
        const f4 bB = *(const f4*)(b1s + j * 32 + 16 + g * 4);
#pragma unroll
        for (int im = 0; im < NIMG; ++im) {
            float hv[8];
#pragma unroll
            for (int r = 0; r < 4; ++r) {
                hv[r] = a1[im][0][r] + bA[r];
                hv[4 + r] = a1[im][1][r] + bB[r];
            }
            gelu_fast_n<8>(hv);
            v8 pf;
#pragma unroll
            for (int r = 0; r < 8; ++r) pf[r] = sat16<T>(hv[r]);
            *(v8*)(smH + im * H_B + j * 1024) = pf;
            if (c == 3 && im == NIMG - 1) { FVIT_CT8_STAMP(9, pf) }
        }
    }
    __syncthreads();
    FVIT_CT8_STAMP(10, xf[0][0])

    {
        f4 acc2[NIMG][2];
#pragma unroll
        for (int im = 0; im < NIMG; ++im) { acc2[im][0] = (f4){0.f, 0.f, 0.f, 0.f}; acc2[im][1] = (f4){0.f, 0.f, 0.f, 0.f}; }
#pragma unroll
        for (int q = 0; q < 8; ++q) {
            v8 hb4[NIMG][4];
#pragma unroll
            for (int im = 0; im < NIMG; ++im)
#pragma unroll
                for (int i = 0; i < 4; ++i) hb4[im][i] = *(const v8*)(smH + im * H_B + (4 * q + i) * 1024);
#pragma unroll
            for (int term = 0; term < WT; ++term) {
                const int t = T_FC2 + q * WT + term;
#pragma unroll
                for (int i = 0; i < 8; ++i)
#pragma unroll
                    for (int im = 0; im < NIMG; ++im) acc2[im][i & 1] = Op16<T>::mfma(ring[t % DEPTH][i], hb4[im][i >> 1], acc2[im][i & 1]);
                __builtin_amdgcn_sched_barrier(0);
                FVIT_CT8_LOAD(t + DEPTH)
            }
        }
        FVIT_CT8_STAMP(11, acc2[NIMG - 1][1])
#pragma unroll
        for (int im = 0; im < NIMG; ++im) {
            if (row_ok && img0 + im < p.B) {
                float* pr = p.R + ((size_t)(img0 + im) * p.G + s) * C;
#pragma unroll
                for (int q = 0; q < 2; ++q) {
                    const int cb = 2 * wave + q;
                    const int co = (cb >> 2) * 64 + g * 16 + (cb & 3) * 4;
                    const f4 bv = *(const f4*)(vecs + 6 * C + co);
                    const f4 gl = *(const f4*)(vecs + 7 * C + co);
                    f4 o = *(const f4*)(smem + OFF_CT + im * CT_B + cb * 1024 + lane16);
#pragma unroll
                    for (int r = 0; r < 4; ++r) o[r] += gl[r] * (acc2[im][q][r] + bv[r]);
                    *(f4*)(pr + co) = o;
                }
            }
        }
    }
    if constexpr (TS) { asm volatile("s_waitcnt vmcnt(0)" ::: "memory"); }
    FVIT_CT8_STAMP(12, threadIdx.x)
#undef FVIT_CT8_STAMP
#undef FVIT_CT8_LOAD
}

}

bool ctblk_supported(int C, int heads, int G, int hidden) { return C == 256 && heads == 8 && hidden == 1024 && G >= 1 && G <= 16; }

int launch_ctblk(const CtBlkCall& c, hipStream_t stream) {
    if (ablate_skip(16)) return FVIT_OK;
    if (!ctblk_supported(c.C, c.heads, c.G, c.hidden) || c.batch <= 0 || !c.X || !c.src_idx || !c.R || !c.wqkv_f || !c.wproj_f || !c.w1f || !c.w2f ||
        !c.bias || !c.bqkv) {
        set_error("ct_block: unsupported arguments C=%d heads=%d G=%d hidden=%d batch=%d", c.C, c.heads, c.G, c.hidden, c.batch);
        return FVIT_EINVAL;
    }
    CtBlkParams p;
    p.X = c.X; p.src_idx = c.src_idx; p.add = c.add; p.R = c.R; p.rowsA = c.rowsA; p.B = c.batch; p.G = c.G;
    p.ln1_w = c.ln1_w; p.ln1_b = c.ln1_b; p.wqkv_f = c.wqkv_f; p.bqkv = c.bqkv; p.wproj_f = c.wproj_f; p.bproj = c.bproj; p.gamma1 = c.gamma1;
    p.bias = c.bias; p.scale = c.scale;
    p.ln2_w = c.ln2_w; p.ln2_b = c.ln2_b; p.w1f = c.w1f; p.b1 = c.b1; p.w2f = c.w2f; p.b2 = c.b2; p.gamma2 = c.gamma2; p.eps = c.eps;
    const double rows = (double)c.batch * c.G;
    const double flops = rows * (2.0 * c.C * 3 * c.C + 4.0 * c.G * c.C + 2.0 * c.C * c.C + 4.0 * c.C * c.hidden);
    const double bytes = rows * c.C * 8.0 + c.terms * 2.0 * (4.0 * c.C * c.C + 2.0 * c.C * c.hidden);
    ProfScope prof(FVIT_K_ATTN_FUSED, flops, bytes, stream);
    prof_note(tune_get("ct_variant", 3) == 3 ? "ctblk8_kernel<256,G16>" : "ctblk_kernel<256,G16>", c.batch);
    p.touch = tune_get("ct_touch", 0);
    p.ts = (unsigned long long*)c.ts;
    if (c.ts) {
        if (c.dtype != FVIT_F16 || c.terms != 1) { set_error("ct_block timeline: fp16, one weight term only"); return FVIT_EINVAL; }
        hipLaunchKernelGGL((ctblk8_kernel<_Float16, 1, 2, true>), dim3(c.batch), dim3(512), 0, stream, p);
        return check_launch("ctblk8_kernel");
    }
    const int variant = tune_get("ct_variant", 3);
    if (c.terms != 1 && c.terms != 2) { set_error("ct_block: weight terms %d (1 or 2)", c.terms); return FVIT_EINVAL; }
    if (variant == 3) {
        const int depth = tune_get("ct8_depth", 3);
#define FVIT_CT8(T_, WT_) do { \
            if (depth == 2) hipLaunchKernelGGL((ctblk8_kernel<T_, WT_, 2>), dim3(c.batch), dim3(512), 0, stream, p); \
            else if (depth == 4) hipLaunchKernelGGL((ctblk8_kernel<T_, WT_, 4>), dim3(c.batch), dim3(512), 0, stream, p); \
            else hipLaunchKernelGGL((ctblk8_kernel<T_, WT_, 3>), dim3(c.batch), dim3(512), 0, stream, p); } while (0)
        if (c.dtype == FVIT_F16) {
            if (c.terms == 2) FVIT_CT8(_Float16, 2); else FVIT_CT8(_Float16, 1);
        } else if (c.dtype == FVIT_BF16) {
            if (c.terms == 2) FVIT_CT8(__bf16, 2); else FVIT_CT8(__bf16, 1);
#undef FVIT_CT8
        } else { set_error("ct_block: operand dtype %d not supported", c.dtype); return FVIT_EINVAL; }
        return check_launch("ctblk8_kernel");
    }
    if (c.dtype == FVIT_F16 && c.terms == 2) {
        hipLaunchKernelGGL((ctblk_kernel<_Float16, 3, 1, 2>), dim3(c.batch), dim3(256), 0, stream, p);
    } else if (c.dtype == FVIT_F16) {
        if (variant == 1) hipLaunchKernelGGL((ctblk_kernel<_Float16, 2, 2>), dim3(c.batch), dim3(256), 0, stream, p);
        else if (variant == 2) hipLaunchKernelGGL((ctblk_kernel<_Float16, 4, 1>), dim3(c.batch), dim3(256), 0, stream, p);
        else hipLaunchKernelGGL((ctblk_kernel<_Float16, 3, 1>), dim3(c.batch), dim3(256), 0, stream, p);
    } else if (c.dtype == FVIT_BF16) {
        if (c.terms == 2) hipLaunchKernelGGL((ctblk_kernel<__bf16, 3, 1, 2>), dim3(c.batch), dim3(256), 0, stream, p);
        else hipLaunchKernelGGL((ctblk_kernel<__bf16, 3, 1>), dim3(c.batch), dim3(256), 0, stream, p);
    } else { set_error("ct_block: operand dtype %d not supported", c.dtype); return FVIT_EINVAL; }
    return check_launch("ctblk_kernel");
}

}
```

fastervit_amd/csrc/fvit_rows.hip:

```cpp
#include "fvit_common.h"

namespace fvit {

namespace {

struct LnParams {
    const float* srcA;
    const float* srcB;
    const int32_t* src_idx;
    const int32_t* add_idx;
    const float* add;
    float* x_out;
    void* n_out;
    const float* ln_w;
    const float* ln_b;
    float eps;
    int rowsA, rowsB, ldn;
    int rows, rows_per_image, C;
    int lw;
    int lo_off;
};

template <typename T, int MAXV>
__global__ __launch_bounds__(256) void ln_kernel(LnParams p) {
// ... 468 lines not shown
        set_error("window_partition: map %dx%d is not a multiple of the window %d (or C %% 4 != 0)", c.Hp, c.Wp, c.ws);
        return FVIT_EINVAL;
    }
    MapParams p;
    p.map = c.in; p.x = c.x; p.ct = c.ct; p.gamma = nullptr; p.up_idx = nullptr;
    p.batch = c.batch; p.C = c.C; p.Hp = c.Hp; p.Wp = c.Wp; p.H = c.Hp; p.W = c.Wp; p.ws = c.ws;
    p.rows_per_win = c.rows_per_win; p.row_off = c.row_off; p.ncw = c.ncw;
    p.nwx = c.Wp / c.ws; p.nw = (c.Hp / c.ws) * p.nwx;
    const double bytes = (double)c.batch * c.C * c.Hp * c.Wp * (elem_size(c.in.dtype) + 4.0);
    int rc;
    {
        ProfScope prof(FVIT_K_PARTITION, 0.0, bytes, stream);
        rc = launch_map(p, false, stream);
    }
    if (rc) return rc;
    if (c.ct && c.ncw > 0)
        rc = launch_ct_copy(c.x, c.rows_per_win, 0, c.ncw, const_cast<float*>(c.ct), c.batch * p.nw, c.C, 1, stream);
    return rc;
}

int launch_reverse(const ReverseCall& c, hipStream_t stream) {
    if (c.ws <= 0 || (c.Hp % c.ws) || (c.Wp % c.ws) || c.H > c.Hp || c.W > c.Wp) {
        set_error("window_reverse: bad geometry Hp=%d Wp=%d H=%d W=%d ws=%d", c.Hp, c.Wp, c.H, c.W, c.ws);
        return FVIT_EINVAL;
    }
    MapParams p;
    p.map = c.out; p.x = const_cast<float*>(c.x); p.ct = nullptr; p.gamma = c.gamma; p.up_idx = c.up_idx;
    p.batch = c.batch; p.C = c.C; p.Hp = c.Hp; p.Wp = c.Wp; p.H = c.H; p.W = c.W; p.ws = c.ws;
    p.rows_per_win = c.rows_per_win; p.row_off = c.row_off; p.ncw = c.row_off;
    p.nwx = c.Wp / c.ws; p.nw = (c.Hp / c.ws) * p.nwx;
    const double bytes = (double)c.batch * c.C * c.H * c.W * (elem_size(c.out.dtype) + 4.0);
    ProfScope prof(FVIT_K_REVERSE, 0.0, bytes, stream);
    return launch_map(p, true, stream);
}

bool reverse_ln_supported(const ReverseCall& c) {
    const int esz = 2;
    return (c.out.dtype == FVIT_F16 || c.out.dtype == FVIT_BF16) && c.out.stride_c == 1 && c.C % 8 == 0 && c.C <= 512 && ((uintptr_t)c.out.data % 16) == 0 &&
           (c.out.stride_b * esz) % 16 == 0 && (c.out.stride_h * esz) % 16 == 0 && (c.out.stride_w * esz) % 16 == 0;
}

int launch_reverse_ln(const ReverseCall& c, const float* ln_w, const float* ln_b, float eps, hipStream_t stream) {
    if (c.ws <= 0 || (c.Hp % c.ws) || (c.Wp % c.ws) || c.H > c.Hp || c.W > c.Wp || !ln_w || !ln_b) {
        set_error("window_reverse_ln: bad geometry Hp=%d Wp=%d H=%d W=%d ws=%d", c.Hp, c.Wp, c.H, c.W, c.ws);
        return FVIT_EINVAL;
    }
    if (!reverse_ln_supported(c)) {
        set_error("window_reverse_ln: needs a 16-bit channel-contiguous, 16-byte aligned map with C %% 8 == 0 and C <= 512 (C=%d, dtype %d)", c.C, c.out.dtype);
        return FVIT_EINVAL;
    }
    MapParams p;
    p.map = c.out; p.x = const_cast<float*>(c.x); p.ct = nullptr; p.gamma = c.gamma; p.up_idx = c.up_idx;
    p.batch = c.batch; p.C = c.C; p.Hp = c.Hp; p.Wp = c.Wp; p.H = c.H; p.W = c.W; p.ws = c.ws;
    p.rows_per_win = c.rows_per_win; p.row_off = c.row_off; p.ncw = c.row_off;
    p.nwx = c.Wp / c.ws; p.nw = (c.Hp / c.ws) * p.nwx;
    const int64_t pix = (int64_t)c.batch * c.H * c.W;
    const int grid = (int)((pix + 3) / 4);
    ProfScope prof(FVIT_K_REVERSE, 8.0 * pix * c.C, (double)pix * c.C * (2.0 + 4.0), stream);
    prof_note("map_rows_ln_cl_kernel", grid);
    if (c.out.dtype == FVIT_F16) hipLaunchKernelGGL((map_rows_ln_cl_kernel<_Float16>), dim3(grid), dim3(256), 0, stream, p, ln_w, ln_b, eps);
    else hipLaunchKernelGGL((map_rows_ln_cl_kernel<__bf16>), dim3(grid), dim3(256), 0, stream, p, ln_w, ln_b, eps);
    return check_launch("window_reverse_ln");
}

int launch_rows_avgpool(const float* x, float* out, int batch, int rows, int C, int round_dtype, hipStream_t stream) {
    if (!x || !out || batch <= 0 || rows <= 0 || C <= 0 || (C % 4) || (round_dtype != FVIT_F16 && round_dtype != FVIT_BF16)) {
        set_error("rows_avgpool: unsupported arguments batch=%d rows=%d C=%d dtype=%d (C %% 4 == 0, a 16-bit map type)", batch, rows, C, round_dtype);
        return FVIT_EINVAL;
    }
    const dim3 grid((C + 255) / 256, batch);
    ProfScope prof(FVIT_K_OTHER, (double)batch * rows * C, 4.0 * batch * C * (rows + 1.0), stream);
    prof_note("rows_avgpool_kernel", (int)(grid.x * grid.y));
    if (round_dtype == FVIT_F16) hipLaunchKernelGGL((rows_avgpool_kernel<_Float16>), grid, dim3(256), 0, stream, x, out, rows, C);
    else hipLaunchKernelGGL((rows_avgpool_kernel<__bf16>), grid, dim3(256), 0, stream, x, out, rows, C);
    return check_launch("rows_avgpool_kernel");
}

int launch_ct_copy(float* x, int rows_per_win, int row_off, int ncw, float* ct, int nwin_total, int C, int to_x,
                   hipStream_t stream) {
    const int64_t nrows = (int64_t)nwin_total * ncw;
    const int C4 = C / 4;
    const int64_t n = nrows * C4;
    ProfScope prof(FVIT_K_OTHER, 0.0, 8.0 * nrows * C, stream);
    hipLaunchKernelGGL(ct_rows_kernel, dim3((unsigned)((n + 255) / 256)), dim3(256), 0, stream, x, ct, rows_per_win, row_off, ncw,
                       nrows, C4, to_x);
    return check_launch("ct_rows_kernel");
}

int launch_token_init(const FvitMapView& in, const float* w, const float* bias, float* out, int B, int C, int Hp, int Wp, int kh, int kw,
                      int sh, int sw, int cw, hipStream_t stream) {
    TokParams p;
    p.in = in; p.w = w; p.bias = bias; p.out = out; p.B = B; p.C = C; p.Hp = Hp; p.Wp = Wp;
    p.kh = kh; p.kw = kw; p.sh = sh; p.sw = sw; p.cw = cw;
    p.Ho = (Hp - kh) / sh + 1;
    p.Wo = (Wp - kw) / sw + 1;
    if (kh <= 0 || kw <= 0 || sh <= 0 || sw <= 0 || cw <= 0 || p.Ho <= 0 || p.Wo <= 0 || (p.Ho % cw) || (p.Wo % cw)) {
        set_error("token_init: bad pooling geometry k=%dx%d s=%dx%d on %dx%d (cw=%d)", kh, kw, sh, sw, Hp, Wp, cw);
        return FVIT_EINVAL;
    }
    const int64_t n = (int64_t)B * p.Ho * p.Wo * C;
    ProfScope prof(FVIT_K_OTHER, 0.0, (double)B * C * Hp * Wp * 2.0 + 4.0 * n, stream);
    const dim3 grid((unsigned)((n + 255) / 256));
    const bool small_patch = kh + 2 <= 8 && kw + 2 <= 8;
#define FVIT_TOK(IN_) do { if (small_patch) hipLaunchKernelGGL((token_init_kernel<IN_, true>), grid, dim3(256), 0, stream, p); \
                           else hipLaunchKernelGGL((token_init_kernel<IN_, false>), grid, dim3(256), 0, stream, p); } while (0)
    if (in.dtype == FVIT_F32) FVIT_TOK(float);
    else if (in.dtype == FVIT_F16) FVIT_TOK(_Float16);
    else if (in.dtype == FVIT_BF16) FVIT_TOK(__bf16);
    else { set_error("token_init: map dtype %d not supported", in.dtype); return FVIT_EINVAL; }
#undef FVIT_TOK
    return check_launch("token_init_kernel");
}

int launch_propagate(float* x, const float* gamma, const int32_t* up_idx, int rows_per_win, int ncw, int nloc, int nwin_total,
                     int C, hipStream_t stream) {
    const int C4 = C / 4;
    const int64_t n = (int64_t)nwin_total * nloc * C4;
    ProfScope prof(FVIT_K_OTHER, 0.0, 12.0 * nwin_total * nloc * (double)C, stream);
    hipLaunchKernelGGL(propagate_kernel, dim3((unsigned)((n + 255) / 256)), dim3(256), 0, stream, x, gamma, up_idx, rows_per_win, ncw,
                       nloc, (int64_t)nwin_total, C4);
    return check_launch("propagate_kernel");
}

}
```

fastervit_amd/csrc/fvit_winblk.hip:

```cpp
#include "fvit_common.h"

namespace fvit {

namespace {

struct WinBlkParams {
    const float* srcA;
    const float* srcB;
    const int32_t* src_idx;
    const int32_t* add_idx;
    const float* add;
    const float* ln_w;
    const float* ln_b;
    float eps;
    int rowsA, rowsB, rows_per_image;
    const void* wqkv_f;
    const float* bqkv;
    const void* wproj_f;
    const float* bproj;
    const float* gamma;
    const float* bias;
    float* x_out;
    int nwin, S;
    float scale;
    float* slab;
    int* counters;
};

template <int CC, int NSPLIT>
constexpr int winblk_lds_bytes() { return 4 * (CC / 32) * 1024 + 4 * (CC / 32 / NSPLIT) * 1024 + (CC / 32) * 96 * 4; }

template <typename T, int CC, int NWV, int NSPLIT = 1, int WT = 1>
__device__ __forceinline__ void winblk_body(const WinBlkParams& p, char* const smem, const int blk) {
    typedef typename Op16<T>::v8 v8;
    constexpr int C = CC, KK = C / 32, CB = C / 16, HEADS = C / 32, NW = NWV, NRB = 4, SP = 64;
    constexpr int HW = HEADS / NSPLIT;
    constexpr int NH = HW / NW;
    static_assert(HW == NH * NW && NH >= 1 && CB == 4 * NW, "heads split evenly over the waves; four output channel blocks per wave");
    constexpr int KQ = KK * WT, PW = HW * WT;
    constexpr int SPH = KQ + 4;
    constexpr size_t QKV_IMG = (size_t)3 * C * C * 2, PROJ_IMG = (size_t)C * C * 2;
    constexpr int DEPTH = 2;
    constexpr int OFF_O = NRB * KK * 1024;
    constexpr int OFF_BQ = OFF_O + NRB * HW * 1024;
    static_assert(OFF_BQ + HEADS * 96 * 4 == winblk_lds_bytes<CC, NSPLIT>(), "LDS layout");
    float* bqs = (float*)(smem + OFF_BQ);

    const int tid = threadIdx.x;
    const int lane = tid & 63;
    const int wave = __builtin_amdgcn_readfirstlane(tid >> 6);
    const int g = lane >> 4, s = lane & 15;
    const int lane16 = lane * 16;
    int win = blk, sp = 0;
    if constexpr (NSPLIT > 1) {
        const int xcd = blk & 7, j = blk >> 3;
        win = (j / NSPLIT) * 8 + xcd;
        sp = j % NSPLIT;
        if (win >= p.nwin) return;
    }
    const int h0 = sp * HW;

    const char* Wq = (const char*)p.wqkv_f + lane16;
    const char* Wp = (const char*)p.wproj_f + lane16;
    const char* Bz = (const char*)p.bias + (s * SP + g * 4) * 4;
    v8 ring[DEPTH][6];
    auto load_qkv = [&](int slot, int h, int u) {
        const char* base = Wq + (u / KK) * QKV_IMG;
        const int kk = u % KK;
#pragma unroll
        for (int ub = 0; ub < 6; ++ub) ring[slot][ub] = *(const v8*)(base + (((size_t)h * 6 + ub) * KK + kk) * 1024);
    };
    auto load_bias = [&](int slot, int h, int qb) {
#pragma unroll
        for (int kb = 0; kb < 4; ++kb) ring[slot][kb] = *(const v8*)(Bz + ((size_t)(h * SP + qb * 16) * SP + kb * 16) * 4);
    };
    auto load_proj = [&](int slot, int hp) {
        const char* base = Wp + (hp / HW) * PROJ_IMG;
        const int h = h0 + hp % HW;
#pragma unroll
        for (int q = 0; q < 4; ++q) ring[slot][q] = *(const v8*)(base + ((size_t)h * CB + 4 * wave + q) * 1024);
    };
    auto issue = [&](int t) {
        if (t < NH * SPH) {
            const int hh = t / SPH, u = t - hh * SPH, h = h0 + NH * wave + hh;
            if (u < KQ) load_qkv(t % DEPTH, h, u);
            else load_bias(t % DEPTH, h, u - KQ);
        } else if (t < NH * SPH + PW) {
            load_proj(t % DEPTH, t - NH * SPH);
        }
        __builtin_amdgcn_sched_barrier(0);
    };

    for (int i = tid; i < HEADS * 96; i += 64 * NW) bqs[i] = p.bqkv[i];
    __builtin_amdgcn_sched_barrier(0);
#pragma unroll
    for (int t = 0; t < DEPTH; ++t) issue(t);

    {
        constexpr int WPR = NW / NRB, KP = KK / WPR;
        const int rb = wave / WPR, part = wave % WPR;
        const int tok = rb * 16 + s;
        const int64_t row = (int64_t)win * p.S + (tok < p.S ? tok : p.S - 1);
        const int b = (int)(row / p.rows_per_image), pr = (int)(row - (int64_t)b * p.rows_per_image);
        const float* src;
        if (p.src_idx) {
            const int si = p.src_idx[pr];
            src = si >= 0 ? p.srcA + ((size_t)b * p.rowsA + si) * C : p.srcB + ((size_t)b * p.rowsB + (-si - 1)) * C;
        } else {
            src = p.srcA + (size_t)row * C;
        }
        const int ai = p.add ? (p.add_idx ? p.add_idx[pr] : pr) : -1;
        const bool has_add = ai >= 0;
        const float* addp = has_add ? p.add + (size_t)ai * C : src;
        f4 v[2 * KK];
        float sum = 0.f;
#pragma unroll
        for (int i = 0; i < 2 * KK; ++i) {
            const int co = (i >> 2) * 64 + g * 16 + (i & 3) * 4;
            f4 t = *(const f4*)(src + co);
            const f4 a = *(const f4*)(addp + co);
#pragma unroll
            for (int r = 0; r < 4; ++r) t[r] += has_add ? a[r] : 0.f;
            v[i] = t;
            sum += (t[0] + t[1]) + (t[2] + t[3]);
        }
        sum = sum_xor32(sum_xor16(sum));
        const float mean = sum / (float)C;
        float sq = 0.f;
#pragma unroll
        for (int i = 0; i < 2 * KK; ++i) {
            const f4 d = v[i] - mean;
            sq += (d[0] * d[0] + d[1] * d[1]) + (d[2] * d[2] + d[3] * d[3]);
        }
        sq = sum_xor32(sum_xor16(sq));
        const float rstd = rsqrtf(sq / (float)C + p.eps);
#pragma unroll
        for (int k8 = 0; k8 < KP; ++k8) {
            v8 o;
#pragma unroll
            for (int h2 = 0; h2 < 2; ++h2) {
                f4 xs = v[2 * k8 + h2];
#pragma unroll
                for (int pp = 1; pp < WPR; ++pp) xs = part == pp ? v[2 * (k8 + pp * KP) + h2] : xs;
                const int kk = k8 + part * KP;
                const int co = (kk >> 1) * 64 + g * 16 + (kk & 1) * 8 + h2 * 4;
                const f4 w = *(const f4*)(p.ln_w + co);
                const f4 bb = *(const f4*)(p.ln_b + co);
#pragma unroll
                for (int r = 0; r < 4; ++r) o[h2 * 4 + r] = sat16<T>((xs[r] - mean) * rstd * w[r] + bb[r]);
            }
            *(v8*)(smem + ((rb * KK + k8 + part * KP) * 1024) + lane16) = o;
        }
    }
    __syncthreads();

    const char* xn = smem + lane16;
#pragma unroll
    for (int hh = 0; hh < NH; ++hh) {
        const int h = h0 + NH * wave + hh;
        f4 acc[6][NRB];
#pragma unroll
        for (int ub = 0; ub < 6; ++ub)
#pragma unroll
            for (int rb = 0; rb < NRB; ++rb) acc[ub][rb] = (f4){0.f, 0.f, 0.f, 0.f};
#pragma unroll
        for (int u = 0; u < KQ; ++u) {
            const int t = hh * SPH + u, kk = u % KK;
            v8 xb[NRB];
#pragma unroll
            for (int rb = 0; rb < NRB; ++rb) xb[rb] = *(const v8*)(xn + (rb * KK + kk) * 1024);
#pragma unroll
            for (int ub = 0; ub < 6; ++ub)
#pragma unroll
                for (int rb = 0; rb < NRB; ++rb)
                    acc[ub][rb] = ub < 4 ? Op16<T>::mfma(ring[t % DEPTH][ub], xb[rb], acc[ub][rb])
                                         : Op16<T>::mfma(xb[rb], ring[t % DEPTH][ub], acc[ub][rb]);
            __builtin_amdgcn_sched_barrier(0);
            issue(t + DEPTH);
        }
        const float* bq = bqs + h * 96;
        v8 qf[NRB], kf[NRB], vf[2][2];
#pragma unroll
        for (int blk = 0; blk < 2; ++blk) {
            const f4 bqv = *(const f4*)(bq + blk * 16 + g * 4);
            const f4 bkv = *(const f4*)(bq + 32 + blk * 16 + g * 4);
#pragma unroll
            for (int rb = 0; rb < NRB; ++rb)
#pragma unroll
                for (int r = 0; r < 4; ++r) {
                    qf[rb][blk * 4 + r] = sat16<T>(acc[blk][rb][r] + bqv[r]);
                    kf[rb][blk * 4 + r] = sat16<T>(acc[2 + blk][rb][r] + bkv[r]);
                }
        }
#pragma unroll
        for (int db = 0; db < 2; ++db) {
            const float bv = bq[64 + db * 16 + s];
#pragma unroll
            for (int k32 = 0; k32 < 2; ++k32)
#pragma unroll
                for (int r = 0; r < 4; ++r) {
                    vf[db][k32][r] = sat16<T>(acc[4 + db][2 * k32][r] + bv);
                    vf[db][k32][4 + r] = sat16<T>(acc[4 + db][2 * k32 + 1][r] + bv);
// ... 41 lines not shown
#pragma unroll
                for (int db = 0; db < 2; ++db) o[db] = Op16<T>::mfma(vf[db][k32], pf, o[db]);
            }
            v8 of;
#pragma unroll
            for (int r = 0; r < 4; ++r) {
                of[r] = sat16<T>(o[0][r] * inv);
                of[4 + r] = sat16<T>(o[1][r] * inv);
            }
            *(v8*)(smem + OFF_O + ((qb * HW + (h - h0)) * 1024) + lane16) = of;
        }
    }
    __syncthreads();

    f4 oacc[4][NRB];
#pragma unroll
    for (int q = 0; q < 4; ++q)
#pragma unroll
        for (int rb = 0; rb < NRB; ++rb) oacc[q][rb] = (f4){0.f, 0.f, 0.f, 0.f};
#pragma unroll
    for (int hp = 0; hp < PW; ++hp) {
        const int t = NH * SPH + hp, h = hp % HW;
        v8 ob[NRB];
#pragma unroll
        for (int rb = 0; rb < NRB; ++rb) ob[rb] = *(const v8*)(xn + OFF_O + (rb * HW + h) * 1024);
#pragma unroll
        for (int q = 0; q < 4; ++q)
#pragma unroll
            for (int rb = 0; rb < NRB; ++rb) oacc[q][rb] = Op16<T>::mfma(ring[t % DEPTH][q], ob[rb], oacc[q][rb]);
        __builtin_amdgcn_sched_barrier(0);
        issue(t + DEPTH);
    }

    if constexpr (NSPLIT > 1) {
        f4* const slab_w = (f4*)p.slab + (size_t)win * NSPLIT * NW * 16 * 64;
        {
            f4* mine = slab_w + ((size_t)sp * NW + wave) * 16 * 64 + lane;
#pragma unroll
            for (int q = 0; q < 4; ++q)
#pragma unroll
                for (int rb = 0; rb < NRB; ++rb) mine[(q * NRB + rb) * 64] = oacc[q][rb];
        }
        asm volatile("s_waitcnt vmcnt(0)" ::: "memory");
        __syncthreads();
        int* const tick = (int*)(smem + OFF_BQ);
        if (tid == 0) {
            __builtin_amdgcn_fence(__ATOMIC_RELEASE, "agent");
            asm volatile("s_waitcnt vmcnt(0)" ::: "memory");
            *tick = __hip_atomic_fetch_add(p.counters + win, 1, __ATOMIC_RELAXED, __HIP_MEMORY_SCOPE_AGENT);
        }
        __syncthreads();
        if (*tick != NSPLIT - 1) return;
        if (tid == 0) {
            __builtin_amdgcn_fence(__ATOMIC_ACQUIRE, "agent");
            p.counters[win] = 0;
        }
        __syncthreads();
#pragma unroll
        for (int q = 0; q < 4; ++q) {
            f4 part[NSPLIT][NRB];
#pragma unroll
            for (int s2 = 0; s2 < NSPLIT; ++s2)
#pragma unroll
                for (int rb = 0; rb < NRB; ++rb) part[s2][rb] = slab_w[(((size_t)s2 * NW + wave) * 16 + q * NRB + rb) * 64 + lane];
#pragma unroll
            for (int rb = 0; rb < NRB; ++rb) {
                f4 sum = part[0][rb];
#pragma unroll
                for (int s2 = 1; s2 < NSPLIT; ++s2) sum += part[s2][rb];
                oacc[q][rb] = sum;
            }
        }
    }

    const bool has_g = p.gamma != nullptr;
    const int c0 = wave * 64 + g * 16;
#pragma unroll
    for (int rb = 0; rb < NRB; ++rb) {
        const int tok = rb * 16 + s;
        if (tok < p.S) {
            const int64_t row = (int64_t)win * p.S + tok;
            const int b = (int)(row / p.rows_per_image), pr = (int)(row - (int64_t)b * p.rows_per_image);
            const float* src;
            if (p.src_idx) {
                const int si = p.src_idx[pr];
                src = si >= 0 ? p.srcA + ((size_t)b * p.rowsA + si) * C : p.srcB + ((size_t)b * p.rowsB + (-si - 1)) * C;
            } else {
                src = p.srcA + (size_t)row * C;
            }
            const int ai = p.add ? (p.add_idx ? p.add_idx[pr] : pr) : -1;
            float* px = p.x_out + (size_t)row * C + c0;
#pragma unroll
            for (int q = 0; q < 4; ++q) {
                f4 xv = *(const f4*)(src + c0 + q * 4);
                if (ai >= 0) xv += *(const f4*)(p.add + (size_t)ai * C + c0 + q * 4);
                const f4 bv = *(const f4*)(p.bproj + c0 + q * 4);
                const f4 gl = *(const f4*)((has_g ? p.gamma : p.bproj) + c0 + q * 4);
#pragma unroll
                for (int r = 0; r < 4; ++r) xv[r] += (has_g ? gl[r] : 1.f) * (oacc[q][rb][r] + bv[r]);
                *(f4*)(px + q * 4) = xv;
            }
        }
    }
}

template <typename T, int CC, int NWV, int NSPLIT = 1, int WT = 1>
__global__ __launch_bounds__(64 * NWV, NWV == 8 ? 1 : 2) void winblk_kernel(WinBlkParams p) {
    __shared__ __attribute__((aligned(16))) char smem[winblk_lds_bytes<CC, NSPLIT>()];
    winblk_body<T, CC, NWV, NSPLIT, WT>(p, smem, blockIdx.x);
}

inline WinBlkParams make_winblk_params(const AttnBlkCall& c) {
    WinBlkParams p;
    p.srcA = c.srcA; p.srcB = c.srcB; p.src_idx = c.src_idx; p.add_idx = c.add_idx; p.add = c.add; p.ln_w = c.ln_w; p.ln_b = c.ln_b; p.eps = c.eps;
    p.rowsA = c.rowsA; p.rowsB = c.rowsB; p.rows_per_image = c.rows_per_image > 0 ? c.rows_per_image : 1;
    p.wqkv_f = c.wqkv_f; p.bqkv = c.bqkv; p.wproj_f = c.wproj_f; p.bproj = c.bproj; p.gamma = c.gamma; p.bias = c.bias; p.x_out = c.x_out;
    p.nwin = c.nwin; p.S = c.S; p.scale = c.scale;
    p.slab = c.slab; p.counters = c.counters;
    return p;
}

}

#ifndef FVIT_BODIES_ONLY
bool winblk_supported(int C, int heads, int S) { return ((C == 512 && heads == 16) || (C == 256 && heads == 8)) && S > 48 && S <= 64; }

int launch_winblk(const AttnBlkCall& c, hipStream_t stream) {
    if (!winblk_supported(c.C, c.heads, c.S) || c.nwin <= 0 || !c.wqkv_f || !c.wproj_f || !c.x_out || !c.bias || !c.bqkv) {
        set_error("win_block: unsupported arguments C=%d heads=%d S=%d nwin=%d", c.C, c.heads, c.S, c.nwin);
        return FVIT_EINVAL;
    }
    if (ablate_skip(4)) return FVIT_OK;
    const WinBlkParams p = make_winblk_params(c);
    if (c.terms != 1 && !(c.terms == 2 && c.C == 512)) {
        set_error("win_block: weight terms %d with C = %d (two-term weights: C = 512 only)", c.terms, c.C);
        return FVIT_EINVAL;
    }
    const bool split = c.C == 512 && c.terms == 1 && c.nsplit == 2 && c.slab && c.counters;
    const double rows = (double)c.nwin * c.S;
    const double flops = rows * (2.0 * c.C * 3 * c.C + 4.0 * c.S * c.C + 2.0 * c.C * c.C);
    const double bytes = rows * c.C * 8.0 + c.terms * 2.0 * 4.0 * c.C * c.C;
    ProfScope prof(FVIT_K_ATTN_FUSED, flops, bytes, stream);
    const int grid = split ? (c.nwin + 7) / 8 * 8 * 2 : c.nwin;
    prof_note(c.C == 512 ? (split ? "winblk_kernel<512,S64,split2>" : "winblk_kernel<512,S64>") : "winblk_kernel<256,S64>", grid);
    if (c.dtype != FVIT_F16 && c.dtype != FVIT_BF16) { set_error("win_block: operand dtype %d not supported", c.dtype); return FVIT_EINVAL; }
    if (c.terms == 2) {
        if (c.dtype == FVIT_F16) hipLaunchKernelGGL((winblk_kernel<_Float16, 512, 8, 1, 2>), dim3(c.nwin), dim3(512), 0, stream, p);
        else hipLaunchKernelGGL((winblk_kernel<__bf16, 512, 8, 1, 2>), dim3(c.nwin), dim3(512), 0, stream, p);
    } else if (split) {
        if (c.dtype == FVIT_F16) hipLaunchKernelGGL((winblk_kernel<_Float16, 512, 8, 2>), dim3(grid), dim3(512), 0, stream, p);
        else hipLaunchKernelGGL((winblk_kernel<__bf16, 512, 8, 2>), dim3(grid), dim3(512), 0, stream, p);
    } else if (c.C == 512) {
        if (c.dtype == FVIT_F16) hipLaunchKernelGGL((winblk_kernel<_Float16, 512, 8>), dim3(c.nwin), dim3(512), 0, stream, p);
        else hipLaunchKernelGGL((winblk_kernel<__bf16, 512, 8>), dim3(c.nwin), dim3(512), 0, stream, p);
    } else {
        if (c.dtype == FVIT_F16) hipLaunchKernelGGL((winblk_kernel<_Float16, 256, 4>), dim3(c.nwin), dim3(256), 0, stream, p);
        else hipLaunchKernelGGL((winblk_kernel<__bf16, 256, 4>), dim3(c.nwin), dim3(256), 0, stream, p);
    }
    return check_launch("winblk_kernel");
}

#endif

}
```

fastervit_amd/csrc/fvit_winmlp.hip:

```cpp
#include "fvit_common.h"

namespace fvit {

namespace {

struct WinMlpParams {
    float* x;
    const float* ln_w;
    const float* ln_b;
    const void* w1f;
    const float* b1;
    const void* w2f;
    const float* b2;
    const float* gamma;
    float eps;
    int M;
    float* slab;
    int* counters;
    unsigned long long* ts;
    int ablate;
};

template <bool TS>
__device__ __forceinline__ void stamp(const WinMlpParams& p, int wave, int lane, int nw, int k) {
    if constexpr (TS) {
        if (p.ts && lane == 0) p.ts[((size_t)blockIdx.x * nw + wave) * 16 + (k < 15 ? k : 15)] = __builtin_amdgcn_s_memtime();
    }
}

constexpr bool winmlp_one_per_cu(int NWV, int NRB) { return NWV == 8 || NRB == 8; }
template <int CC, int HID, int NRB, int NWV>
constexpr int winmlp_lds_bytes() {
    constexpr int hbuf = (NRB * (CC / 32) + 2 * NWV * NRB) * 1024 + HID * 4 <= (winmlp_one_per_cu(NWV, NRB) ? 150 : 72) * 1024 ? 2 : 1;
    return NRB * (CC / 32) * 1024 + hbuf * NWV * NRB * 1024 + HID * 4;
}

template <typename T, int CC, int HID, int NRB, int DEPTH, int NWV = 8, int SP = 1, int NSPLIT = 1, bool TS = false, bool PIPE = false>
__device__ __forceinline__ void winmlp_body(const WinMlpParams& p, char* const smem, const int blk) {
    typedef typename Op16<T>::v8 v8;
    constexpr int C = CC, KK = C / 32, CB = C / 16, NW = NWV;
    constexpr int CBW = CB / NW;
    constexpr int NSC = HID / 32 / NW / NSPLIT;
    static_assert(HID % (32 * NW * NSPLIT) == 0, "hidden units must split evenly");
    constexpr int F1S = 2 * KK / 8;
    constexpr int CPS = 8 / CBW;
    constexpr int F2S = NW / CPS;
    constexpr int F1T = SP * F1S, F2T = SP * F2S;
    constexpr int SPS = F1T + F2T;
    constexpr size_t WBYTES = (size_t)HID * C * 2;
    static_assert(SPS % DEPTH == 0, "ring slots must be static inside the super-chunk loop");
    static_assert(CBW % 2 == 0, "a wave owns whole k steps of XN");
    constexpr int HBUF = (NRB * KK + 2 * NW * NRB) * 1024 + HID * 4 <= (winmlp_one_per_cu(NW, NRB) ? 150 : 72) * 1024 ? 2 : 1;
    constexpr int OFF_H = NRB * KK * 1024;
    constexpr int OFF_B1 = OFF_H + HBUF * NW * NRB * 1024;
    static_assert(OFF_B1 + HID * 4 == winmlp_lds_bytes<CC, HID, NRB, NWV>(), "LDS layout");
    static_assert(2 * NRB * 64 * CB * 4 <= HBUF * NW * NRB * 1024, "the row statistics of phase A fit in the H region");
    float* b1s = (float*)(smem + OFF_B1);

    const int tid = threadIdx.x;
    const int lane = tid & 63;
    const int wave = __builtin_amdgcn_readfirstlane(tid >> 6);
    const int g = lane >> 4, s = lane & 15;
    const int lane16 = lane * 16;
    int rg = blk, sp = 0;
    if constexpr (NSPLIT > 1) {
        const int xcd = blk & 7, j = blk >> 3;
        rg = (j / NSPLIT) * 8 + xcd;
        sp = j % NSPLIT;
        if (rg * (16 * NRB) >= p.M) return;
    }
    const int row0 = rg * (16 * NRB);
    const int sc0 = sp * NSC;

    stamp<TS>(p, wave, lane, NWV, 0);
    const char* W1 = (const char*)p.w1f + lane16;
    const char* W2 = (const char*)p.w2f + lane16;
    v8 ring[DEPTH][8];
#ifdef FVIT_DIAG
    const bool abl_w = p.ablate & 1, abl_b = p.ablate & 2, abl_g = p.ablate & 4;
#else
    constexpr bool abl_w = false, abl_b = false, abl_g = false;
#endif
    bool in_loop = false;
    auto issue = [&](int sc, int u, int slot) {
        if (sc < NSC && !(abl_w && in_loop)) {
            if (u < F1T) {
                const int uu = u % F1S;
                const char* b = W1 + (size_t)(u / F1S) * WBYTES + (size_t)((sc0 + sc) * NW + wave) * 2 * KK * 1024;
#pragma unroll
                for (int i = 0; i < 8; ++i) ring[slot][i] = *(const v8*)(b + ((i & 1) * KK + 4 * uu + (i >> 1)) * 1024);
            } else {
                const int vv = (u - F1T) % F2S;
                const char* b = W2 + (size_t)((u - F1T) / F2S) * WBYTES + ((size_t)((sc0 + sc) * NW + CPS * vv) * CB + CBW * wave) * 1024;
#pragma unroll
                for (int i = 0; i < 8; ++i) ring[slot][i] = *(const v8*)(b + ((i / CBW) * CB + (i % CBW)) * 1024);
            }
        }
        __builtin_amdgcn_sched_barrier(0);
    };

    constexpr int NT = 64 * NW;
    float c1[HID / NT];
#pragma unroll
    for (int i = 0; i < HID / NT; ++i) c1[i] = p.b1[tid + NT * i];
    __builtin_amdgcn_sched_barrier(0);
#pragma unroll
    for (int t = 0; t < DEPTH; ++t) issue(0, t, t);
    in_loop = true;
    f4 acc2[CBW][NRB], lnw[CBW], lnb[CBW];
#pragma unroll
    for (int rb = 0; rb < NRB; ++rb) {
        const int row = min(row0 + rb * 16 + s, p.M - 1);
#pragma unroll
        for (int q = 0; q < CBW; ++q) {
            const int cb = CBW * wave + q;
            acc2[q][rb] = *(const f4*)(p.x + (size_t)row * C + (cb >> 2) * 64 + g * 16 + (cb & 3) * 4);
        }
    }
#pragma unroll
    for (int q = 0; q < CBW; ++q) {
// ... 214 lines not shown
            if (has_next) fc1(sc + 1, false);
            if (!abl_b) __syncthreads();
            const int hbuf = sc & 1;
            const char* hr = smem + OFF_H + hbuf * NW * NRB * 1024 + lane16;
            const int jn = min((sc0 + sc + 1) * NW + wave, HID / 32 - 1);
#pragma unroll
            for (int v = 0; v < F2T; ++v) {
#pragma unroll
                for (int c = 0; c < CPS; ++c) {
                    v8 hb4[NRB];
#pragma unroll
                    for (int rb = 0; rb < NRB; ++rb) hb4[rb] = *(const v8*)(hr + ((CPS * (v % F2S) + c) * NRB + rb) * 1024);
#pragma unroll
                    for (int q = 0; q < CBW; ++q)
#pragma unroll
                        for (int rb = 0; rb < NRB; ++rb) acc2[q][rb] = Op16<T>::mfma(ring[v % DEPTH][c * CBW + q], hb4[rb], acc2[q][rb]);
                }
#pragma unroll
                for (int rb = v * NRB / F2T; rb < (v + 1) * NRB / F2T; ++rb) gelu_publish(jn, hbuf ^ 1, rb);
                __builtin_amdgcn_sched_barrier(0);
                const int nv = v + DEPTH;
                if (nv < F2T) load_f2(v % DEPTH, sc, nv);
                else if (sc + 2 < NSC) load_f1(v % DEPTH, sc + 2, nv - F2T);
                else load_f2(v % DEPTH, sc + 1, nv - F2T);
            }
            stamp<TS>(p, wave, lane, NWV, sc + 4 < 13 ? sc + 4 : 13);
        }
    }
    stamp<TS>(p, wave, lane, NWV, 14);

    if constexpr (NSPLIT > 1) {
        constexpr int FPW = CBW * NRB;
        f4* const slab_rg = (f4*)p.slab + (size_t)rg * NSPLIT * NW * FPW * 64;
        {
            f4* mine = slab_rg + ((size_t)sp * NW + wave) * FPW * 64 + lane;
#pragma unroll
            for (int q = 0; q < CBW; ++q)
#pragma unroll
                for (int rb = 0; rb < NRB; ++rb) mine[(q * NRB + rb) * 64] = acc2[q][rb];
        }
        asm volatile("s_waitcnt vmcnt(0)" ::: "memory");
        __syncthreads();
        int* const tick = (int*)(smem + OFF_B1);
        if (tid == 0) {
            __builtin_amdgcn_fence(__ATOMIC_RELEASE, "agent");
            asm volatile("s_waitcnt vmcnt(0)" ::: "memory");
            *tick = __hip_atomic_fetch_add(p.counters + rg, 1, __ATOMIC_RELAXED, __HIP_MEMORY_SCOPE_AGENT);
        }
        __syncthreads();
        if (*tick != NSPLIT - 1) return;
        if (tid == 0) {
            __builtin_amdgcn_fence(__ATOMIC_ACQUIRE, "agent");
            p.counters[rg] = 0;
        }
        __syncthreads();
#pragma unroll
        for (int q = 0; q < CBW; ++q) {
#pragma unroll
            for (int rh = 0; rh < NRB; rh += 2) {
                f4 part[NSPLIT][2];
#pragma unroll
                for (int s2 = 0; s2 < NSPLIT; ++s2)
#pragma unroll
                    for (int r2 = 0; r2 < 2; ++r2) part[s2][r2] = slab_rg[(((size_t)s2 * NW + wave) * FPW + q * NRB + rh + r2) * 64 + lane];
#pragma unroll
                for (int r2 = 0; r2 < 2; ++r2) {
                    f4 sum = part[0][r2];
#pragma unroll
                    for (int s2 = 1; s2 < NSPLIT; ++s2) sum += part[s2][r2];
                    acc2[q][rh + r2] = sum;
                }
            }
        }
    }

    f4 bvq[CBW];
#pragma unroll
    for (int q = 0; q < CBW; ++q) {
        const int cb = CBW * wave + q;
        bvq[q] = *(const f4*)(p.b2 + (cb >> 2) * 64 + g * 16 + (cb & 3) * 4);
    }
    int row0e = row0;
    asm volatile("" : "+s"(row0e));
    if (acc_from_x) {
#pragma unroll
        for (int rb = 0; rb < NRB; ++rb) {
            const int row = row0e + rb * 16 + s;
            if (row < p.M) {
#pragma unroll
                for (int q = 0; q < CBW; ++q) {
                    const int cb = CBW * wave + q;
                    const int pk = xh[q][rb];
                    const f4 hi = {__builtin_amdgcn_cvt_f32_bf8(pk, 0), __builtin_amdgcn_cvt_f32_bf8(pk, 1), __builtin_amdgcn_cvt_f32_bf8(pk, 2),
                                   __builtin_amdgcn_cvt_f32_bf8(pk, 3)};
                    *(f4*)(p.x + (size_t)row * C + (cb >> 2) * 64 + g * 16 + (cb & 3) * 4) = hi + (acc2[q][rb] + bvq[q]);
                }
            }
        }
    } else {
        const bool has_g = p.gamma != nullptr;
        f4 glq[CBW], xv[NRB][CBW];
#pragma unroll
        for (int q = 0; q < CBW; ++q) {
            const int cb = CBW * wave + q;
            glq[q] = *(const f4*)((has_g ? p.gamma : p.b2) + (cb >> 2) * 64 + g * 16 + (cb & 3) * 4);
        }
#pragma unroll
        for (int rb = 0; rb < NRB; ++rb) {
            const int row = min(row0e + rb * 16 + s, p.M - 1);
#pragma unroll
            for (int q = 0; q < CBW; ++q) {
                const int cb = CBW * wave + q;
                xv[rb][q] = *(const f4*)(p.x + (size_t)row * C + (cb >> 2) * 64 + g * 16 + (cb & 3) * 4);
            }
        }
        __builtin_amdgcn_sched_barrier(0);
#pragma unroll
        for (int rb = 0; rb < NRB; ++rb) {
            const int row = row0e + rb * 16 + s;
            if (row < p.M) {
#pragma unroll
                for (int q = 0; q < CBW; ++q) {
                    const int cb = CBW * wave + q;
                    f4 o = xv[rb][q];
#pragma unroll
                    for (int r = 0; r < 4; ++r) o[r] += (has_g ? glq[q][r] : 1.f) * (acc2[q][rb][r] + bvq[q][r]);
                    *(f4*)(p.x + (size_t)row * C + (cb >> 2) * 64 + g * 16 + (cb & 3) * 4) = o;
                }
            }
        }
    }
    if constexpr (TS) {
        asm volatile("s_waitcnt vmcnt(0)" ::: "memory");
        stamp<TS>(p, wave, lane, NWV, 15);
    }
}

template <typename T, int CC, int HID, int NRB, int DEPTH, int NWV = 8, int SP = 1, int NSPLIT = 1, bool TS = false, bool PIPE = false>
__global__ __launch_bounds__(64 * NWV, winmlp_one_per_cu(NWV, NRB) ? 1 : 2) void winmlp_kernel(WinMlpParams p) {
    __shared__ __attribute__((aligned(16))) char smem[winmlp_lds_bytes<CC, HID, NRB, NWV>()];
    winmlp_body<T, CC, HID, NRB, DEPTH, NWV, SP, NSPLIT, TS, PIPE>(p, smem, blockIdx.x);
}

inline WinMlpParams make_winmlp_params(const MlpFusedCall& c) {
    WinMlpParams p;
    p.x = c.x; p.ln_w = c.ln_w; p.ln_b = c.ln_b; p.w1f = c.w1f; p.b1 = c.b1; p.w2f = c.w2f; p.b2 = c.b2; p.gamma = c.gamma; p.eps = c.eps; p.M = c.M;
    p.slab = c.slab; p.counters = c.counters; p.ts = (unsigned long long*)c.ts;
    p.ablate = diag_knob("wm_ablate");
    return p;
}

}

#ifndef FVIT_BODIES_ONLY
size_t winmlp_split_slab_bytes(int64_t M, int C, int nsplit) { return (size_t)((M + 63) / 64) * (size_t)nsplit * 64 * C * 4; }

bool winmlp_supported(int C, int hidden) { return (C == 512 && hidden == 2048) || (C == 256 && hidden == 1024); }

int launch_winmlp(const MlpFusedCall& c, hipStream_t stream) {
    if (!winmlp_supported(c.C, c.hidden) || c.M <= 0 || !c.x || !c.w1f || !c.w2f) {
        set_error("win_mlp: unsupported arguments C=%d hidden=%d M=%d", c.C, c.hidden, c.M);
        return FVIT_EINVAL;
    }
    if (ablate_skip(c.C == 512 ? 2 : 1)) return FVIT_OK;
    const WinMlpParams p = make_winmlp_params(c);
    const int nsplit = (c.C == 512 && c.slab && c.counters && c.nsplit == 2) ? 2 : 1;
    const double flops = 4.0 * c.M * (double)c.C * c.hidden;
    const double bytes = 8.0 * c.M * (double)c.C + 4.0 * c.C * (double)c.hidden;
    ProfScope prof(FVIT_K_MLP_FUSED, flops, bytes, stream);
    const int form256 = c.C == 256 && !c.ts ? tune_get("win_mlp256", 2) : 2;
    const bool wide256 = form256 == 1;
    const int rows_per_wg = wide256 ? 128 : 64;
    const int nrg = (c.M + rows_per_wg - 1) / rows_per_wg;
    const int grid = nsplit > 1 ? (nrg + 7) / 8 * 8 * nsplit : nrg;
    prof_note(c.C == 512 ? (nsplit == 2 ? "winmlp_kernel<512,split2>" : "winmlp_kernel<512>")
                         : (wide256 ? "winmlp_kernel<256,128rows>" : "winmlp_kernel<256>"), grid);
    if (c.dtype != FVIT_F16 && c.dtype != FVIT_BF16) { set_error("win_mlp: operand dtype %d not supported", c.dtype); return FVIT_EINVAL; }
    if (c.terms != 1 && c.terms != 2) { set_error("win_mlp: weight terms %d not supported", c.terms); return FVIT_EINVAL; }
#define FVIT_WINMLP(T, CC_, HID_, NRB_, NWV_, SP_) \
    hipLaunchKernelGGL((winmlp_kernel<T, CC_, HID_, NRB_, 2, NWV_, SP_>), dim3(grid), dim3(64 * NWV_), 0, stream, p)
#define FVIT_WINMLP_T(CC_, HID_, NRB_, NWV_)                                                     \
    do {                                                                                         \
        if (c.dtype == FVIT_F16) { if (c.terms == 2) FVIT_WINMLP(_Float16, CC_, HID_, NRB_, NWV_, 2); else FVIT_WINMLP(_Float16, CC_, HID_, NRB_, NWV_, 1); } \
        else { if (c.terms == 2) FVIT_WINMLP(__bf16, CC_, HID_, NRB_, NWV_, 2); else FVIT_WINMLP(__bf16, CC_, HID_, NRB_, NWV_, 1); } \
    } while (0)
#define FVIT_WINMLP_P(T, CC_, HID_, NRB_, NWV_, SP_) \
    hipLaunchKernelGGL((winmlp_kernel<T, CC_, HID_, NRB_, 2, NWV_, SP_, 1, false, true>), dim3(grid), dim3(64 * NWV_), 0, stream, p)
#define FVIT_WINMLP_PT(CC_, HID_, NRB_, NWV_)                                                    \
    do {                                                                                         \
        if (c.dtype == FVIT_F16) { if (c.terms == 2) FVIT_WINMLP_P(_Float16, CC_, HID_, NRB_, NWV_, 2); else FVIT_WINMLP_P(_Float16, CC_, HID_, NRB_, NWV_, 1); } \
        else { if (c.terms == 2) FVIT_WINMLP_P(__bf16, CC_, HID_, NRB_, NWV_, 2); else FVIT_WINMLP_P(__bf16, CC_, HID_, NRB_, NWV_, 1); } \
    } while (0)
    const int pipe = tune_get("win_mlp_pipe", 1);
#define FVIT_WINMLP_S(T, SP_, NS_) hipLaunchKernelGGL((winmlp_kernel<T, 512, 2048, 4, 2, 8, SP_, NS_>), dim3(grid), dim3(512), 0, stream, p)
#define FVIT_WINMLP_ST(NS_)                                                                      \
    do {                                                                                         \
        if (c.dtype == FVIT_F16) { if (c.terms == 2) FVIT_WINMLP_S(_Float16, 2, NS_); else FVIT_WINMLP_S(_Float16, 1, NS_); } \
        else { if (c.terms == 2) FVIT_WINMLP_S(__bf16, 2, NS_); else FVIT_WINMLP_S(__bf16, 1, NS_); } \
    } while (0)
#ifdef FVIT_DIAG
    if (c.ts && c.dtype == FVIT_F16 && c.terms == 1 && nsplit == 1) {
        if (c.C == 512) hipLaunchKernelGGL((winmlp_kernel<_Float16, 512, 2048, 4, 2, 8, 1, 1, true>), dim3(grid), dim3(512), 0, stream, p);
        else hipLaunchKernelGGL((winmlp_kernel<_Float16, 256, 1024, 4, 2, 4, 1, 1, true>), dim3(grid), dim3(256), 0, stream, p);
    } else
#endif
    if (c.C == 512 && nsplit == 2) FVIT_WINMLP_ST(2);
    else if (c.C == 512 && pipe) FVIT_WINMLP_PT(512, 2048, 4, 8);
    else if (c.C == 512) FVIT_WINMLP_T(512, 2048, 4, 8);
    else if (wide256) FVIT_WINMLP_T(256, 1024, 8, 8);
    else FVIT_WINMLP_T(256, 1024, 4, 4);
#undef FVIT_WINMLP_ST
#undef FVIT_WINMLP_S
#undef FVIT_WINMLP_PT
#undef FVIT_WINMLP_P
#undef FVIT_WINMLP_T
#undef FVIT_WINMLP
    return check_launch("winmlp_kernel");
}

#endif

}
```

Before: 92610 images/s.

## Fuse stage-entry partition into first attention block and stage-exit LayerNorm into last MLP

```diff
diff --git a/fastervit_amd/csrc/fvit_api.hip b/fastervit_amd/csrc/fvit_api.hip
--- a/fastervit_amd/csrc/fvit_api.hip
+++ b/fastervit_amd/csrc/fvit_api.hip
@@ -226,6 +226,12 @@
     bool preadd_eligible = false;
     const float* pe_next = nullptr;
     int win_blk_split = 1, win_mlp_split = 1;
+    RowMap entry_map;
+    const float* entry_ct = nullptr;
+    RowMap exit_map;
+    const float* exit_ln_w = nullptr;
+    const float* exit_ln_b = nullptr;
+    float exit_eps = 0.f;
 };
 
 struct RouteKnobs {
@@ -237,6 +243,7 @@
     const int win_mlp = tune_get("win_mlp", 1), win_mlp256 = tune_get("win_mlp256", 2), win_mlp_split = tune_get("win_mlp_split", 1);
     const int win_fused = tune_get("win_fused", 1), win_fused256 = tune_get("win_fused256", 0), win_blk_split = tune_get("win_blk_split", 1);
     const int ct_fused = tune_get("ct_fused", 1), pe_preadd = tune_get("pe_preadd", 1);
+    const int stage_entry_fused = tune_get("stage_entry_fused", 1), stage_exit_fused = tune_get("stage_exit_fused", 1);
 };
 
 static BlockRoute choose_route(const FvitStageDesc& d, const StageLayout& L, const FvitBlockWeights& w, const RouteKnobs& k) {
@@ -336,8 +343,10 @@
             mc.counters = (int*)(ws + L.off_CNT);
             mc.nsplit = r.win_mlp_split;
         }
+        const bool exits = r.exit_map.data && b.rows == L.Mx;
+        if (exits) { mc.out_map = r.exit_map; mc.out_ln_w = r.exit_ln_w; mc.out_ln_b = r.exit_ln_b; mc.out_eps = r.exit_eps; }
         FVIT_TRY(launch_winmlp(mc, st));
-        dbg_rowhash("winmlp.out", b.x, b.rows, d.C * 4, st);
+        if (!exits) dbg_rowhash("winmlp.out", b.x, b.rows, d.C * 4, st);
         return FVIT_OK;
     }
     case MlpRoute::MLP_FUSED: {
@@ -377,6 +386,62 @@
                                   a.w_qkv_frag, a.b_qkv_heads, a.w_proj_frag, a.b_proj, a.gamma, a.bias, X, d.batch * L.nW, L.S, d.heads, d.C, L.scale);
     ab.terms = d.weight_terms;
     return ab;
+}
+
+static MlpFusedCall window_mlp_call(const FvitStageDesc& d, const StageLayout& L, const FvitMlpWeights& w, float* X) {
+    MlpFusedCall mc = mlp_fused_call(d.operand_dtype, X, (int)L.Mx, d.C, d.hidden, w.ln_w, w.ln_b, 1e-5f, w.w_fc1_frag, w.b_fc1, w.w_fc2_frag, w.b_fc2, w.gamma);
+    mc.terms = d.weight_terms;
+    return mc;
+}
+
+static RowMap row_map(const FvitStageDesc& d, const StageLayout& L, const FvitMapView& m) {
+    RowMap r;
+    r.data = m.data; r.stride_b = m.stride_b; r.stride_h = m.stride_h; r.stride_w = m.stride_w; r.bf16 = m.dtype == FVIT_BF16;
+    r.S = L.S; r.ncw = L.ncw; r.ws = d.ws; r.nwx = d.Wp / d.ws; r.nw = L.nW;
+    return r;
+}
+static bool map_16bit_cl(const FvitMapView& m, int align_bytes) {
+    return (m.dtype == FVIT_F16 || m.dtype == FVIT_BF16) && m.stride_c == 1 && ((uintptr_t)m.data % align_bytes) == 0 && (m.stride_b * 2) % align_bytes == 0 &&
+           (m.stride_h * 2) % align_bytes == 0 && (m.stride_w * 2) % align_bytes == 0;
+}
+
+static AttnBlkCall window_winblk_call(const FvitStageDesc& d, const StageLayout& L, const BlockRoute& r, const FvitBlockWeights& w, const FvitStageTables& t,
+                                      float* X, float* R, char* ws) {
+    AttnBlkCall ab = window_attnblk_call(d, L, w, t, X, R);
+    if (L.off_SLAB) {
+        ab.slab = (float*)(ws + L.off_SLAB);
+        ab.counters = (int*)(ws + L.off_CNT);
+        ab.nsplit = r.win_blk_split;
+    }
+    return ab;
+}
+
+static void choose_stage_boundaries(const FvitStageDesc& d, const StageLayout& L, const FvitBlockWeights* blocks, const FvitStageTables& t, const FvitMapView& in,
+                                    const float* ct_init, const FvitMapView* out, const FvitStageTail* tail, bool prop, const ReverseCall& rc,
+                                    const RouteKnobs& k, char* ws, std::vector<BlockRoute>& routes) {
+    if (d.depth <= 0 || d.H != d.Hp || d.W != d.Wp || prop) return;
+    for (int i = 0; i < d.depth; ++i)
+        if (blocks[i].attn.gamma || blocks[i].mlp.gamma || (d.hier && (blocks[i].hat_attn.gamma || blocks[i].hat_mlp.gamma))) return;
+    float* X = (float*)(ws + L.off_X);
+    float* R = (float*)(ws + L.off_R);
+    BlockRoute& first = routes[0];
+    if (k.stage_entry_fused && map_16bit_cl(in, 8) && d.C % 4 == 0 && d.weight_terms <= 2) {
+        bool ok = false;
+        if (first.window_attn == WinAttnRoute::ATTNBLK) ok = attnblk_map_source_supported(window_attnblk_call(d, L, blocks[0], t, X, R));
+        else if (first.window_attn == WinAttnRoute::WINBLK) ok = winblk_map_source_supported(window_winblk_call(d, L, first, blocks[0], t, X, R, ws));
+        if (ok) {
+            first.entry_map = row_map(d, L, in);
+            if (first.carrier == CarrierRoute::FUSED_CT) first.entry_ct = ct_init;
+        }
+    }
+    BlockRoute& last = routes[d.depth - 1];
+    if (k.stage_exit_fused && tail && tail->ln_w && out && reverse_ln_supported(rc) && last.window_mlp == MlpRoute::WINMLP &&
+        winmlp_exit_supported(window_mlp_call(d, L, blocks[d.depth - 1].mlp, X))) {
+        last.exit_map = row_map(d, L, *out);
+        last.exit_ln_w = tail->ln_w;
+        last.exit_ln_b = tail->ln_b;
+        last.exit_eps = tail->ln_eps;
+    }
 }
 
 static int run_block(const FvitStageDesc& d, const StageLayout& L, const BlockRoute& r, const FvitBlockWeights& w, const FvitStageTables& t,
@@ -400,6 +465,7 @@
                                   ha.b_qkv_heads, ha.w_proj_frag, ha.b_proj, ha.gamma, ha.bias, L.scale, hm.ln_w, hm.ln_b, hm.w_fc1_frag, hm.b_fc1,
                                   hm.w_fc2_frag, hm.b_fc2, hm.gamma, 1e-5f);
         cb.terms = d.weight_terms;
+        if (r.entry_ct) { cb.X = r.entry_ct; cb.rowsA = L.G; cb.src_S = L.S; cb.src_ncw = L.ncw; }
         FVIT_TRY(launch_ctblk(cb, st));
         dbg_rowhash("ct.block", R, L.Mc, d.C * 4, st);
         break;
@@ -428,20 +494,19 @@
     const FvitAttnWeights& a = w.attn;
     switch (r.window_attn) {
     case WinAttnRoute::WINBLK: {
-        AttnBlkCall ab = window_attnblk_call(d, L, w, t, X, R);
-        if (L.off_SLAB) {
-            ab.slab = (float*)(ws + L.off_SLAB);
-            ab.counters = (int*)(ws + L.off_CNT);
-            ab.nsplit = r.win_blk_split;
-        }
+        AttnBlkCall ab = window_winblk_call(d, L, r, w, t, X, R, ws);
+        ab.map = r.entry_map;
         FVIT_TRY(launch_winblk(ab, st));
         dbg_rowhash("win.winblk", X, L.Mx, d.C * 4, st);
         break;
     }
-    case WinAttnRoute::ATTNBLK:
-        FVIT_TRY(launch_attnblk(window_attnblk_call(d, L, w, t, X, R), st));
+    case WinAttnRoute::ATTNBLK: {
+        AttnBlkCall ab = window_attnblk_call(d, L, w, t, X, R);
+        ab.map = r.entry_map;
+        FVIT_TRY(launch_attnblk(ab, st));
         dbg_rowhash("win.attnblk", X, L.Mx, d.C * 4, st);
         break;
+    }
     case WinAttnRoute::LNGEMM_PREADDED: {
         LnGemmCall lg = {ln_call(d, L, a.ln_w, a.ln_b, X, L.Mx, nullptr), a.w_qkv, L.ldn, a.b_qkv, win.qkv, L.ldqkv, L.ldqkv, 0};
         FVIT_TRY(launch_ln_gemm(lg, st));
@@ -548,9 +613,6 @@
     hipStream_t st = (hipStream_t)stream;
     char* ws = (char*)workspace;
     float* X = (float*)(ws + L.off_X);
-    PartitionCall pc = {*in, d.batch, d.C, d.Hp, d.Wp, d.ws, X, L.S, L.ncw, d.hier ? ct_init : nullptr, L.ncw};
-    FVIT_TRY(launch_partition(pc, st));
-    dbg_rowhash("partition", X, L.Mx, d.C * 4, st);
     const RouteKnobs knobs{};
     std::vector<BlockRoute> routes;
     for (int i = 0; i < d.depth; ++i) routes.push_back(choose_route(d, L, blocks[i], knobs));
@@ -560,12 +622,21 @@
             routes[i + 1].window_attn = WinAttnRoute::LNGEMM_PREADDED;
         }
     }
+    const bool prop = d.hier && d.do_propagation && d.depth > 0 && blocks[d.depth - 1].last;
+    ReverseCall rc = {X, L.S, L.ncw, d.batch, d.C, d.Hp, d.Wp, d.H, d.W, d.ws, out ? *out : FvitMapView{},
+                      prop ? blocks[d.depth - 1].hat_attn.gamma : nullptr, prop ? tables->up_idx : nullptr};
+    choose_stage_boundaries(d, L, blocks, *tables, *in, ct_init, out, tail, prop, rc, knobs, ws, routes);
+    if (d.depth > 0 && routes[0].entry_map.data) {
+        if (d.hier && !routes[0].entry_ct) FVIT_TRY(launch_ct_copy(X, L.S, 0, L.ncw, const_cast<float*>(ct_init), d.batch * L.nW, d.C, 1, st));
+    } else {
+        PartitionCall pc = {*in, d.batch, d.C, d.Hp, d.Wp, d.ws, X, L.S, L.ncw, d.hier ? ct_init : nullptr, L.ncw};
+        FVIT_TRY(launch_partition(pc, st));
+        dbg_rowhash("partition", X, L.Mx, d.C * 4, st);
+    }
     for (int i = 0; i < d.depth; ++i) FVIT_TRY(run_block(d, L, routes[i], blocks[i], *tables, ws, st));
+    if (d.depth > 0 && routes[d.depth - 1].exit_map.data) return FVIT_OK;
     if (pooled)
         return launch_rows_avgpool(X, tail->pool_out, d.batch, L.S, d.C, tail->pool_dtype, st);
-    const bool prop = d.hier && d.do_propagation && d.depth > 0 && blocks[d.depth - 1].last;
-    ReverseCall rc = {X, L.S, L.ncw, d.batch, d.C, d.Hp, d.Wp, d.H, d.W, d.ws, *out,
-                      prop ? blocks[d.depth - 1].hat_attn.gamma : nullptr, prop ? tables->up_idx : nullptr};
     if (tail && tail->ln_w) return launch_reverse_ln(rc, tail->ln_w, tail->ln_b, tail->ln_eps, st);
     FVIT_TRY(launch_reverse(rc, st));
     return FVIT_OK;
diff --git a/fastervit_amd/csrc/fvit_attnblk.hip b/fastervit_amd/csrc/fvit_attnblk.hip
--- a/fastervit_amd/csrc/fvit_attnblk.hip
+++ b/fastervit_amd/csrc/fvit_attnblk.hip
@@ -25,6 +25,7 @@
     float scale;
     int ablate;
     unsigned long long* ts;
+    RowMap map;
     int stagger;
 };
 
@@ -33,7 +34,7 @@
                                      (__attribute__((address_space(3))) void*)lds_dst, 16, 0, 0);
 }
 
-template <typename T, int CC, int NRB, int NW, bool BIAS_LDS, bool DBQ = false, bool TS = false, int WT = 1>
+template <typename T, int CC, int NRB, int NW, bool BIAS_LDS, bool DBQ = false, bool TS = false, int WT = 1, bool MAPSRC = false>
 __global__ __launch_bounds__(64 * NW, (CC == 256 && WT == 1) ? 2 : 1) void attnblk_kernel(AttnBlkParams p) {
     static_assert(WT == 1 || (WT == 2 && DBQ && !BIAS_LDS && !TS), "two weight terms: DBQ form, bias from L2");
     typedef typename Op16<T>::v8 v8;
@@ -113,30 +114,47 @@
 
     const float* src;
     const float* addp = nullptr;
+    const char* mpx = nullptr;
     {
         const int b = (int)(row / p.rows_per_image), pr = (int)(row - (int64_t)b * p.rows_per_image);
         if (p.src_idx) {
             const int si = p.src_idx[pr];
             src = si >= 0 ? p.srcA + ((size_t)b * p.rowsA + si) * C : p.srcB + ((size_t)b * p.rowsB + (-si - 1)) * C;
+            if constexpr (MAPSRC) {
+                if (si >= 0) mpx = rowmap_px(p.map, (int64_t)b * p.rowsA + si);
+            }
         } else {
             src = p.srcA + (size_t)row * C;
+            if constexpr (MAPSRC) mpx = rowmap_px(p.map, row);
         }
         if (p.add) {
             const int ai = p.add_idx ? p.add_idx[pr] : pr;
             if (ai >= 0) addp = p.add + (size_t)ai * C;
         }
     }
+    auto load_row = [&](f4 (&xr)[2 * KK]) {
+        auto co = [&](int i) { return (i >> 2) * 64 + g * 16 + ((i >> 1) & 1) * 8 + (i & 1) * 4; };
+        if constexpr (MAPSRC) {
+            if (mpx) { rowmap_load_row(xr, mpx, p.map.bf16, co); return; }
+        }
+#pragma unroll
+        for (int i = 0; i < 2 * KK; ++i) xr[i] = *(const f4*)(src + co(i));
+    };
     constexpr bool KEEPX = CC == 256;
     v8 xf[KK];
     f4 v[KK][2];
     {
         float sum = 0.f;
+        f4 xr[2 * KK];
+        if constexpr (MAPSRC) load_row(xr);
 #pragma unroll
         for (int kk = 0; kk < KK; ++kk)
 #pragma unroll
             for (int h2 = 0; h2 < 2; ++h2) {
                 const int co = (kk >> 1) * 64 + g * 16 + (kk & 1) * 8 + h2 * 4;
-                f4 t = *(const f4*)(src + co);
+                f4 t;
+                if constexpr (MAPSRC) t = xr[2 * kk + h2];
+                else t = *(const f4*)(src + co);
                 if (addp) t += *(const f4*)(addp + co);
                 v[kk][h2] = t;
                 sum += (t[0] + t[1]) + (t[2] + t[3]);
@@ -349,6 +367,8 @@
 
     if (row_ok) {
         float* px = p.x_out + (size_t)row * C;
+        f4 xr[2 * KK];
+        if constexpr (MAPSRC && !KEEPX) load_row(xr);
 #pragma unroll
         for (int cg = 0; cg < CB / 4; ++cg) {
             const int c0 = cg * 64 + g * 16;
@@ -358,7 +378,8 @@
                 if (KEEPX) {
                     xv = v[2 * cg + (q >> 1)][q & 1];
                 } else {
-                    xv = *(const f4*)(src + c0 + q * 4);
+                    if constexpr (MAPSRC) xv = xr[2 * (2 * cg + (q >> 1)) + (q & 1)];
+                    else xv = *(const f4*)(src + c0 + q * 4);
                     if (addp) xv += *(const f4*)(addp + c0 + q * 4);
                 }
                 const f4 bv = *(const f4*)(bps + c0 + q * 4);
@@ -380,6 +401,10 @@
 bool attnblk_supported(int C, int heads, int S) {
     if (C == 256 && heads == 8) return (S >= 1 && S <= 16) || (S > 48 && S <= 64);
     return C == 512 && heads == 16 && S > 48 && S <= 64;
+}
+
+bool attnblk_map_source_supported(const AttnBlkCall& c) {
+    return c.C == 256 && c.heads == 8 && c.S > 48 && c.S <= 64 && !c.ts && (c.terms == 2 || (c.terms == 1 && tune_get("ab_variant", 0) == 0));
 }
 
 int launch_attnblk(const AttnBlkCall& c, hipStream_t stream) {
@@ -396,9 +421,15 @@
     p.ablate = diag_knob("ab_ablate");
     p.stagger = tune_get("ab_stagger", 0);
     p.ts = (unsigned long long*)c.ts;
+    p.map = c.map;
+    const bool mapsrc = c.map.data != nullptr;
+    if (mapsrc && !attnblk_map_source_supported(c)) {
+        set_error("attn_block: no map-source instance for C=%d S=%d terms=%d in this form", c.C, c.S, c.terms);
+        return FVIT_EINVAL;
+    }
     const double rows = (double)c.nwin * c.S;
     const double flops = 2.0 * rows * c.C * 4.0 * c.C + 4.0 * c.nwin * (double)c.heads * c.S * (double)c.S * 32.0;
-    const double bytes = 8.0 * rows * c.C + 8.0 * c.C * c.C;
+    const double bytes = (mapsrc ? 6.0 : 8.0) * rows * c.C + 8.0 * c.C * c.C;
     ProfScope prof(FVIT_K_ATTN_FUSED, flops, bytes, stream);
     prof_note(c.C == 256 ? (c.S <= 16 ? "attnblk_kernel<256,S16>" : "attnblk_kernel<256,S64>") : "attnblk_kernel<512,S64>", c.nwin);
     const bool small = c.S <= 16;
@@ -410,7 +441,12 @@
     if (c.terms == 2) {
         prof_note("attnblk_kernel<256,S64,2 terms>", (c.nwin + 1) / 2);
         if (c.ts) { set_error("attn_block timeline: one weight term only"); return FVIT_EINVAL; }
-        if (c.dtype == FVIT_F16) hipLaunchKernelGGL((attnblk_kernel<_Float16, 256, 4, 8, false, true, false, 2>), dim3((c.nwin + 1) / 2), dim3(512), 0, stream, p);
+        if (c.dtype != FVIT_F16 && c.dtype != FVIT_BF16) { set_error("attn_block: operand dtype %d not supported", c.dtype); return FVIT_EINVAL; }
+        if (mapsrc) {
+            if (c.dtype == FVIT_F16) hipLaunchKernelGGL((attnblk_kernel<_Float16, 256, 4, 8, false, true, false, 2, true>), dim3((c.nwin + 1) / 2), dim3(512), 0, stream, p);
+            else hipLaunchKernelGGL((attnblk_kernel<__bf16, 256, 4, 8, false, true, false, 2, true>), dim3((c.nwin + 1) / 2), dim3(512), 0, stream, p);
+        }
+        else if (c.dtype == FVIT_F16) hipLaunchKernelGGL((attnblk_kernel<_Float16, 256, 4, 8, false, true, false, 2>), dim3((c.nwin + 1) / 2), dim3(512), 0, stream, p);
         else if (c.dtype == FVIT_BF16) hipLaunchKernelGGL((attnblk_kernel<__bf16, 256, 4, 8, false, true, false, 2>), dim3((c.nwin + 1) / 2), dim3(512), 0, stream, p);
         else { set_error("attn_block: operand dtype %d not supported", c.dtype); return FVIT_EINVAL; }
         return check_launch("attnblk_kernel");
@@ -427,7 +463,11 @@
         hipLaunchKernelGGL((attnblk_kernel<_Float16, 256, 4, 4, false, false, true>), dim3(c.nwin), dim3(256), 0, stream, p);
         return check_launch("attnblk_kernel");
     }
-    if (c.dtype == FVIT_F16) {
+    if (mapsrc) {
+        if (c.dtype == FVIT_F16) hipLaunchKernelGGL((attnblk_kernel<_Float16, 256, 4, 4, false, false, false, 1, true>), dim3(c.nwin), dim3(256), 0, stream, p);
+        else if (c.dtype == FVIT_BF16) hipLaunchKernelGGL((attnblk_kernel<__bf16, 256, 4, 4, false, false, false, 1, true>), dim3(c.nwin), dim3(256), 0, stream, p);
+        else { set_error("attn_block: operand dtype %d not supported", c.dtype); return FVIT_EINVAL; }
+    } else if (c.dtype == FVIT_F16) {
         if (small) FVIT_AB(_Float16, 1, 8, true);
         else if (dbq) FVIT_AB_DBQ(_Float16);
         else if (variant == 1) FVIT_AB(_Float16, 4, 8, true);
diff --git a/fastervit_amd/csrc/fvit_common.h b/fastervit_amd/csrc/fvit_common.h
--- a/fastervit_amd/csrc/fvit_common.h
+++ b/fastervit_amd/csrc/fvit_common.h
@@ -77,6 +77,59 @@
     if constexpr (N >= 32) x = max_xor16(x);
     if constexpr (N >= 64) x = max_xor32(x);
     return x;
+}
+
+struct RowMap {
+    void* data = nullptr;
+    int64_t stride_b = 0, stride_h = 0, stride_w = 0;
+    int bf16 = 0;
+    int S = 0, ncw = 0;
+    int ws = 0, nwx = 0, nw = 0;
+};
+__device__ __forceinline__ int64_t rowmap_pixel(const RowMap& m, int64_t row) {
+    const int64_t win = row / m.S;
+    const int tok = (int)(row - win * m.S) - m.ncw;
+    if (tok < 0) return -1;
+    const int b = (int)(win / m.nw), wi = (int)(win - (int64_t)b * m.nw);
+    const int wy = wi / m.nwx, wx = wi - wy * m.nwx, ty = tok / m.ws, tx = tok - ty * m.ws;
+    return b * m.stride_b + (wy * m.ws + ty) * m.stride_h + (wx * m.ws + tx) * m.stride_w;
+}
+__device__ __forceinline__ const char* rowmap_px(const RowMap& m, int64_t row) {
+    const int64_t off = rowmap_pixel(m, row);
+    return off >= 0 ? (const char*)m.data + 2 * off : nullptr;
+}
+template <typename V4>
+__device__ __forceinline__ f4 rowmap_load4(const void* px) {
+    const V4 v = *(const V4*)px;
+    f4 t;
+#pragma unroll
+    for (int r = 0; r < 4; ++r) t[r] = (float)v[r];
+    return t;
+}
+template <int N, typename OFF>
+__device__ __forceinline__ void rowmap_load_row(f4 (&v)[N], const char* px, int bf16, OFF off) {
+    if (bf16) {
+#pragma unroll
+        for (int i = 0; i < N; ++i) v[i] = rowmap_load4<b4>(px + 2 * off(i));
+    } else {
+#pragma unroll
+        for (int i = 0; i < N; ++i) v[i] = rowmap_load4<h4>(px + 2 * off(i));
+    }
+}
+__device__ __forceinline__ float rowmap_round(float x, int bf16) { return bf16 ? (float)(__bf16)x : (float)(_Float16)x; }
+
+__device__ __forceinline__ void rowmap_store8(void* px, const float (&y)[8], int bf16) {
+    if (bf16) {
+        b8 o;
+#pragma unroll
+        for (int r = 0; r < 8; ++r) o[r] = (__bf16)y[r];
+        *(b8*)px = o;
+    } else {
+        h8 o;
+#pragma unroll
+        for (int r = 0; r < 8; ++r) o[r] = (_Float16)y[r];
+        *(h8*)px = o;
+    }
 }
 
 __device__ __forceinline__ float fast_erf(float x) {
@@ -295,7 +348,12 @@
     int* counters = nullptr;
     int nsplit = 1;
     void* ts = nullptr;
-};
+    RowMap out_map;
+    const float* out_ln_w = nullptr;
+    const float* out_ln_b = nullptr;
+    float out_eps = 0.f;
+};
+bool winmlp_exit_supported(const MlpFusedCall& c);
 size_t winmlp_split_slab_bytes(int64_t M, int C, int nsplit);
 bool mlp_fused_supported(int C, int hidden);
 int launch_mlp_fused(const MlpFusedCall& c, hipStream_t stream);
@@ -329,8 +387,11 @@
     int nsplit = 1;
     int terms = 1;
     void* ts = nullptr;
+    RowMap map;
 };
 bool attnblk_supported(int C, int heads, int S);
+bool attnblk_map_source_supported(const AttnBlkCall& c);
+bool winblk_map_source_supported(const AttnBlkCall& c);
 int launch_attnblk(const AttnBlkCall& c, hipStream_t stream);
 bool attnblk2_supported(int C, int heads, int S);
 int launch_attnblk2(const AttnBlkCall& c, hipStream_t stream);
@@ -388,6 +449,7 @@
     float eps;
     int terms = 1;
     void* ts = nullptr;
+    int src_S = 0, src_ncw = 0;
 };
 bool ctblk_supported(int C, int heads, int G, int hidden);
 int launch_ctblk(const CtBlkCall& c, hipStream_t stream);
diff --git a/fastervit_amd/csrc/fvit_ctblk.hip b/fastervit_amd/csrc/fvit_ctblk.hip
--- a/fastervit_amd/csrc/fvit_ctblk.hip
+++ b/fastervit_amd/csrc/fvit_ctblk.hip
@@ -10,6 +10,7 @@
     const float* add;
     float* R;
     int rowsA, B, G;
+    int src_S, src_ncw;
     const float* ln1_w; const float* ln1_b;
     const void* wqkv_f;
     const float* bqkv;
@@ -27,6 +28,11 @@
     unsigned long long* ts;
 };
 
+__device__ __forceinline__ int ct_src_row(const CtBlkParams& p, int tok) {
+    const int si = p.src_idx[tok];
+    return p.src_S > 0 ? (si / p.src_S) * p.src_ncw + si % p.src_S : si;
+}
+
 template <typename T, int DEPTH, int MINB, int WT = 1>
 __global__ __launch_bounds__(256, MINB) void ctblk_kernel(CtBlkParams p) {
     typedef typename Op16<T>::v8 v8;
@@ -107,7 +113,7 @@
         for (int i = 0; i < 8; ++i) bzs[tid + 256 * i] = c3[i];
     }
 
-    const float* src = p.X + ((size_t)img * p.rowsA + p.src_idx[tok]) * C + g * 16;
+    const float* src = p.X + ((size_t)img * p.rowsA + ct_src_row(p, tok)) * C + g * 16;
     const bool has_add = p.add != nullptr, has_g1 = p.gamma1 != nullptr, has_g2 = p.gamma2 != nullptr;
     const float* addp = has_add ? p.add + (size_t)tok * C + g * 16 : src;
     auto gather = [&](f4 (&v)[CB]) {
@@ -385,7 +391,7 @@
 #pragma unroll
     for (int im = 0; im < NIMG; ++im) {
         const int img = min(img0 + im, p.B - 1);
-        const float* src = p.X + ((size_t)img * p.rowsA + p.src_idx[tok]) * C + g * 16;
+        const float* src = p.X + ((size_t)img * p.rowsA + ct_src_row(p, tok)) * C + g * 16;
 #pragma unroll
         for (int q = 0; q < 2; ++q) {
             const int cb = 2 * wave + q;
@@ -751,6 +757,7 @@
     }
     CtBlkParams p;
     p.X = c.X; p.src_idx = c.src_idx; p.add = c.add; p.R = c.R; p.rowsA = c.rowsA; p.B = c.batch; p.G = c.G;
+    p.src_S = c.src_S; p.src_ncw = c.src_ncw;
     p.ln1_w = c.ln1_w; p.ln1_b = c.ln1_b; p.wqkv_f = c.wqkv_f; p.bqkv = c.bqkv; p.wproj_f = c.wproj_f; p.bproj = c.bproj; p.gamma1 = c.gamma1;
     p.bias = c.bias; p.scale = c.scale;
     p.ln2_w = c.ln2_w; p.ln2_b = c.ln2_b; p.w1f = c.w1f; p.b1 = c.b1; p.w2f = c.w2f; p.b2 = c.b2; p.gamma2 = c.gamma2; p.eps = c.eps;
diff --git a/fastervit_amd/csrc/fvit_rows.hip b/fastervit_amd/csrc/fvit_rows.hip
--- a/fastervit_amd/csrc/fvit_rows.hip
+++ b/fastervit_amd/csrc/fvit_rows.hip
@@ -574,6 +574,7 @@
     const int C4 = C / 4;
     const int64_t n = nrows * C4;
     ProfScope prof(FVIT_K_OTHER, 0.0, 8.0 * nrows * C, stream);
+    prof_note("ct_rows_kernel", (int)((n + 255) / 256));
     hipLaunchKernelGGL(ct_rows_kernel, dim3((unsigned)((n + 255) / 256)), dim3(256), 0, stream, x, ct, rows_per_win, row_off, ncw,
                        nrows, C4, to_x);
     return check_launch("ct_rows_kernel");
diff --git a/fastervit_amd/csrc/fvit_winblk.hip b/fastervit_amd/csrc/fvit_winblk.hip
--- a/fastervit_amd/csrc/fvit_winblk.hip
+++ b/fastervit_amd/csrc/fvit_winblk.hip
@@ -25,12 +25,13 @@
     float scale;
     float* slab;
     int* counters;
+    RowMap map;
 };
 
 template <int CC, int NSPLIT>
 constexpr int winblk_lds_bytes() { return 4 * (CC / 32) * 1024 + 4 * (CC / 32 / NSPLIT) * 1024 + (CC / 32) * 96 * 4; }
 
-template <typename T, int CC, int NWV, int NSPLIT = 1, int WT = 1>
+template <typename T, int CC, int NWV, int NSPLIT = 1, int WT = 1, bool MAPSRC = false>
 __device__ __forceinline__ void winblk_body(const WinBlkParams& p, char* const smem, const int blk) {
     typedef typename Op16<T>::v8 v8;
     constexpr int C = CC, KK = C / 32, CB = C / 16, HEADS = C / 32, NW = NWV, NRB = 4, SP = 64;
@@ -103,21 +104,36 @@
         const int64_t row = (int64_t)win * p.S + (tok < p.S ? tok : p.S - 1);
         const int b = (int)(row / p.rows_per_image), pr = (int)(row - (int64_t)b * p.rows_per_image);
         const float* src;
+        const char* mpx = nullptr;
         if (p.src_idx) {
             const int si = p.src_idx[pr];
             src = si >= 0 ? p.srcA + ((size_t)b * p.rowsA + si) * C : p.srcB + ((size_t)b * p.rowsB + (-si - 1)) * C;
+            if constexpr (MAPSRC) {
+                if (si >= 0) mpx = rowmap_px(p.map, (int64_t)b * p.rowsA + si);
+            }
         } else {
             src = p.srcA + (size_t)row * C;
+            if constexpr (MAPSRC) mpx = rowmap_px(p.map, row);
         }
         const int ai = p.add ? (p.add_idx ? p.add_idx[pr] : pr) : -1;
         const bool has_add = ai >= 0;
         const float* addp = has_add ? p.add + (size_t)ai * C : src;
         f4 v[2 * KK];
         float sum = 0.f;
+        if constexpr (MAPSRC) {
+            if (mpx) {
+                rowmap_load_row(v, mpx, p.map.bf16, [&](int i) { return (i >> 2) * 64 + g * 16 + (i & 3) * 4; });
+            } else {
+#pragma unroll
+                for (int i = 0; i < 2 * KK; ++i) v[i] = *(const f4*)(src + (i >> 2) * 64 + g * 16 + (i & 3) * 4);
+            }
+        }
 #pragma unroll
         for (int i = 0; i < 2 * KK; ++i) {
             const int co = (i >> 2) * 64 + g * 16 + (i & 3) * 4;
-            f4 t = *(const f4*)(src + co);
+            f4 t;
+            if constexpr (MAPSRC) t = v[i];
+            else t = *(const f4*)(src + co);
             const f4 a = *(const f4*)(addp + co);
 #pragma unroll
             for (int r = 0; r < 4; ++r) t[r] += has_add ? a[r] : 0.f;
@@ -325,17 +341,28 @@
             const int64_t row = (int64_t)win * p.S + tok;
             const int b = (int)(row / p.rows_per_image), pr = (int)(row - (int64_t)b * p.rows_per_image);
             const float* src;
+            const char* mpx = nullptr;
             if (p.src_idx) {
                 const int si = p.src_idx[pr];
                 src = si >= 0 ? p.srcA + ((size_t)b * p.rowsA + si) * C : p.srcB + ((size_t)b * p.rowsB + (-si - 1)) * C;
+                if constexpr (MAPSRC) {
+                    if (si >= 0) mpx = rowmap_px(p.map, (int64_t)b * p.rowsA + si);
+                }
             } else {
                 src = p.srcA + (size_t)row * C;
+                if constexpr (MAPSRC) mpx = rowmap_px(p.map, row);
             }
             const int ai = p.add ? (p.add_idx ? p.add_idx[pr] : pr) : -1;
             float* px = p.x_out + (size_t)row * C + c0;
+            f4 xm[4];
+            if constexpr (MAPSRC) {
+                if (mpx) rowmap_load_row(xm, mpx, p.map.bf16, [&](int q) { return c0 + q * 4; });
+            }
 #pragma unroll
             for (int q = 0; q < 4; ++q) {
-                f4 xv = *(const f4*)(src + c0 + q * 4);
+                f4 xv;
+                if (MAPSRC && mpx) xv = xm[q];
+                else xv = *(const f4*)(src + c0 + q * 4);
                 if (ai >= 0) xv += *(const f4*)(p.add + (size_t)ai * C + c0 + q * 4);
                 const f4 bv = *(const f4*)(p.bproj + c0 + q * 4);
                 const f4 gl = *(const f4*)((has_g ? p.gamma : p.bproj) + c0 + q * 4);
@@ -347,10 +374,10 @@
     }
 }
 
-template <typename T, int CC, int NWV, int NSPLIT = 1, int WT = 1>
+template <typename T, int CC, int NWV, int NSPLIT = 1, int WT = 1, bool MAPSRC = false>
 __global__ __launch_bounds__(64 * NWV, NWV == 8 ? 1 : 2) void winblk_kernel(WinBlkParams p) {
     __shared__ __attribute__((aligned(16))) char smem[winblk_lds_bytes<CC, NSPLIT>()];
-    winblk_body<T, CC, NWV, NSPLIT, WT>(p, smem, blockIdx.x);
+    winblk_body<T, CC, NWV, NSPLIT, WT, MAPSRC>(p, smem, blockIdx.x);
 }
 
 inline WinBlkParams make_winblk_params(const AttnBlkCall& c) {
@@ -360,6 +387,7 @@
     p.wqkv_f = c.wqkv_f; p.bqkv = c.bqkv; p.wproj_f = c.wproj_f; p.bproj = c.bproj; p.gamma = c.gamma; p.bias = c.bias; p.x_out = c.x_out;
     p.nwin = c.nwin; p.S = c.S; p.scale = c.scale;
     p.slab = c.slab; p.counters = c.counters;
+    p.map = c.map;
     return p;
 }
 
@@ -367,6 +395,11 @@
 
 #ifndef FVIT_BODIES_ONLY
 bool winblk_supported(int C, int heads, int S) { return ((C == 512 && heads == 16) || (C == 256 && heads == 8)) && S > 48 && S <= 64; }
+
+bool winblk_map_source_supported(const AttnBlkCall& c) {
+    const bool split = c.C == 512 && c.terms == 1 && c.nsplit == 2 && c.slab && c.counters;
+    return winblk_supported(c.C, c.heads, c.S) && !split && (c.terms == 1 || (c.terms == 2 && c.C == 512));
+}
 
 int launch_winblk(const AttnBlkCall& c, hipStream_t stream) {
     if (!winblk_supported(c.C, c.heads, c.S) || c.nwin <= 0 || !c.wqkv_f || !c.wproj_f || !c.x_out || !c.bias || !c.bqkv) {
@@ -382,12 +415,24 @@
     const bool split = c.C == 512 && c.terms == 1 && c.nsplit == 2 && c.slab && c.counters;
     const double rows = (double)c.nwin * c.S;
     const double flops = rows * (2.0 * c.C * 3 * c.C + 4.0 * c.S * c.C + 2.0 * c.C * c.C);
-    const double bytes = rows * c.C * 8.0 + c.terms * 2.0 * 4.0 * c.C * c.C;
+    const bool mapsrc = c.map.data != nullptr;
+    if (mapsrc && !winblk_map_source_supported(c)) {
+        set_error("win_block: no map-source instance for C=%d terms=%d nsplit=%d", c.C, c.terms, c.nsplit);
+        return FVIT_EINVAL;
+    }
+    const double bytes = rows * c.C * (mapsrc ? 6.0 : 8.0) + c.terms * 2.0 * 4.0 * c.C * c.C;
     ProfScope prof(FVIT_K_ATTN_FUSED, flops, bytes, stream);
     const int grid = split ? (c.nwin + 7) / 8 * 8 * 2 : c.nwin;
     prof_note(c.C == 512 ? (split ? "winblk_kernel<512,S64,split2>" : "winblk_kernel<512,S64>") : "winblk_kernel<256,S64>", grid);
     if (c.dtype != FVIT_F16 && c.dtype != FVIT_BF16) { set_error("win_block: operand dtype %d not supported", c.dtype); return FVIT_EINVAL; }
-    if (c.terms == 2) {
+    if (mapsrc) {
+#define FVIT_WB_MAP(T_) do { \
+        if (c.terms == 2) hipLaunchKernelGGL((winblk_kernel<T_, 512, 8, 1, 2, true>), dim3(c.nwin), dim3(512), 0, stream, p); \
+        else if (c.C == 512) hipLaunchKernelGGL((winblk_kernel<T_, 512, 8, 1, 1, true>), dim3(c.nwin), dim3(512), 0, stream, p); \
+        else hipLaunchKernelGGL((winblk_kernel<T_, 256, 4, 1, 1, true>), dim3(c.nwin), dim3(256), 0, stream, p); } while (0)
+        if (c.dtype == FVIT_F16) FVIT_WB_MAP(_Float16); else FVIT_WB_MAP(__bf16);
+#undef FVIT_WB_MAP
+    } else if (c.terms == 2) {
         if (c.dtype == FVIT_F16) hipLaunchKernelGGL((winblk_kernel<_Float16, 512, 8, 1, 2>), dim3(c.nwin), dim3(512), 0, stream, p);
         else hipLaunchKernelGGL((winblk_kernel<__bf16, 512, 8, 1, 2>), dim3(c.nwin), dim3(512), 0, stream, p);
     } else if (split) {
diff --git a/fastervit_amd/csrc/fvit_winmlp.hip b/fastervit_amd/csrc/fvit_winmlp.hip
--- a/fastervit_amd/csrc/fvit_winmlp.hip
+++ b/fastervit_amd/csrc/fvit_winmlp.hip
@@ -18,6 +18,10 @@
     float* slab;
     int* counters;
     unsigned long long* ts;
+    RowMap out_map;
+    const float* out_ln_w;
+    const float* out_ln_b;
+    float out_eps;
     int ablate;
 };
 
@@ -35,7 +39,7 @@
     return NRB * (CC / 32) * 1024 + hbuf * NWV * NRB * 1024 + HID * 4;
 }
 
-template <typename T, int CC, int HID, int NRB, int DEPTH, int NWV = 8, int SP = 1, int NSPLIT = 1, bool TS = false, bool PIPE = false>
+template <typename T, int CC, int HID, int NRB, int DEPTH, int NWV = 8, int SP = 1, int NSPLIT = 1, bool TS = false, bool PIPE = false, bool LNMAP = false>
 __device__ __forceinline__ void winmlp_body(const WinMlpParams& p, char* const smem, const int blk) {
     typedef typename Op16<T>::v8 v8;
     constexpr int C = CC, KK = C / 32, CB = C / 16, NW = NWV;
@@ -416,7 +420,77 @@
     }
     int row0e = row0;
     asm volatile("" : "+s"(row0e));
-    if (acc_from_x) {
+    if constexpr (LNMAP) {
+        static_assert(KEEPX && CBW == 4 && HBUF == 2 && !PIPE && !TS, "the stage-exit epilogue: 4 waves x 16 contiguous channels per lane, plain loop, double-buffered H");
+        const int mb = p.out_map.bf16;
+        float* const st = (float*)(smem + OFF_H + (((NSC - 1) & 1) ^ 1) * NW * NRB * 1024);
+#pragma unroll
+        for (int rb = 0; rb < NRB; ++rb) {
+            float sum = 0.f;
+#pragma unroll
+            for (int q = 0; q < CBW; ++q) {
+                const int pk = xh[q][rb];
+                const f4 hi = {__builtin_amdgcn_cvt_f32_bf8(pk, 0), __builtin_amdgcn_cvt_f32_bf8(pk, 1), __builtin_amdgcn_cvt_f32_bf8(pk, 2),
+                               __builtin_amdgcn_cvt_f32_bf8(pk, 3)};
+                const f4 v = hi + (acc2[q][rb] + bvq[q]);
+#pragma unroll
+                for (int r = 0; r < 4; ++r) acc2[q][rb][r] = rowmap_round(v[r], mb);
+                sum += (acc2[q][rb][0] + acc2[q][rb][1]) + (acc2[q][rb][2] + acc2[q][rb][3]);
+            }
+            sum = sum_xor32(sum_xor16(sum));
+            if (g == 0) st[(rb * NW + wave) * 16 + s] = sum;
+        }
+        __syncthreads();
+        float omean[NRB], orstd[NRB];
+#pragma unroll
+        for (int rb = 0; rb < NRB; ++rb) {
+            float sum = 0.f;
+#pragma unroll
+            for (int w = 0; w < NW; ++w) sum += st[(rb * NW + w) * 16 + s];
+            omean[rb] = sum / (float)C;
+            float sq = 0.f;
+#pragma unroll
+            for (int q = 0; q < CBW; ++q) {
+                const f4 d = acc2[q][rb] - omean[rb];
+                sq += (d[0] * d[0] + d[1] * d[1]) + (d[2] * d[2] + d[3] * d[3]);
+            }
+            sq = sum_xor32(sum_xor16(sq));
+            if (g == 0) st[((NRB + rb) * NW + wave) * 16 + s] = sq;
+        }
+        __syncthreads();
+#pragma unroll
+        for (int rb = 0; rb < NRB; ++rb) {
+            float sq = 0.f;
+#pragma unroll
+            for (int w = 0; w < NW; ++w) sq += st[((NRB + rb) * NW + w) * 16 + s];
+            orstd[rb] = rsqrtf(sq / (float)C + p.out_eps);
+        }
+        const int c0 = wave * 64 + g * 16;
+        f4 ow[CBW], ob[CBW];
+#pragma unroll
+        for (int q = 0; q < CBW; ++q) {
+            ow[q] = *(const f4*)(p.out_ln_w + c0 + q * 4);
+            ob[q] = *(const f4*)(p.out_ln_b + c0 + q * 4);
+        }
+#pragma unroll
+        for (int rb = 0; rb < NRB; ++rb) {
+            const int row = row0e + rb * 16 + s;
+            const int64_t off = rowmap_pixel(p.out_map, min(row, p.M - 1));
+            if (row < p.M && off >= 0) {
+                char* px = (char*)p.out_map.data + 2 * (off + c0);
+#pragma unroll
+                for (int q2 = 0; q2 < CBW / 2; ++q2) {
+                    float y[8];
+#pragma unroll
+                    for (int r = 0; r < 4; ++r) {
+                        y[r] = (acc2[2 * q2][rb][r] - omean[rb]) * orstd[rb] * ow[2 * q2][r] + ob[2 * q2][r];
+                        y[4 + r] = (acc2[2 * q2 + 1][rb][r] - omean[rb]) * orstd[rb] * ow[2 * q2 + 1][r] + ob[2 * q2 + 1][r];
+                    }
+                    rowmap_store8(px + q2 * 16, y, mb);
+                }
+            }
+        }
+    } else if (acc_from_x) {
 #pragma unroll
         for (int rb = 0; rb < NRB; ++rb) {
             const int row = row0e + rb * 16 + s;
@@ -470,16 +544,17 @@
     }
 }
 
-template <typename T, int CC, int HID, int NRB, int DEPTH, int NWV = 8, int SP = 1, int NSPLIT = 1, bool TS = false, bool PIPE = false>
+template <typename T, int CC, int HID, int NRB, int DEPTH, int NWV = 8, int SP = 1, int NSPLIT = 1, bool TS = false, bool PIPE = false, bool LNMAP = false>
 __global__ __launch_bounds__(64 * NWV, winmlp_one_per_cu(NWV, NRB) ? 1 : 2) void winmlp_kernel(WinMlpParams p) {
     __shared__ __attribute__((aligned(16))) char smem[winmlp_lds_bytes<CC, HID, NRB, NWV>()];
-    winmlp_body<T, CC, HID, NRB, DEPTH, NWV, SP, NSPLIT, TS, PIPE>(p, smem, blockIdx.x);
+    winmlp_body<T, CC, HID, NRB, DEPTH, NWV, SP, NSPLIT, TS, PIPE, LNMAP>(p, smem, blockIdx.x);
 }
 
 inline WinMlpParams make_winmlp_params(const MlpFusedCall& c) {
     WinMlpParams p;
     p.x = c.x; p.ln_w = c.ln_w; p.ln_b = c.ln_b; p.w1f = c.w1f; p.b1 = c.b1; p.w2f = c.w2f; p.b2 = c.b2; p.gamma = c.gamma; p.eps = c.eps; p.M = c.M;
     p.slab = c.slab; p.counters = c.counters; p.ts = (unsigned long long*)c.ts;
+    p.out_map = c.out_map; p.out_ln_w = c.out_ln_w; p.out_ln_b = c.out_ln_b; p.out_eps = c.out_eps;
     p.ablate = diag_knob("wm_ablate");
     return p;
 }
@@ -490,6 +565,10 @@
 size_t winmlp_split_slab_bytes(int64_t M, int C, int nsplit) { return (size_t)((M + 63) / 64) * (size_t)nsplit * 64 * C * 4; }
 
 bool winmlp_supported(int C, int hidden) { return (C == 512 && hidden == 2048) || (C == 256 && hidden == 1024); }
+
+bool winmlp_exit_supported(const MlpFusedCall& c) {
+    return c.C == 256 && c.hidden == 1024 && !c.gamma && !c.ts && (c.terms == 1 || c.terms == 2) && tune_get("win_mlp256", 2) == 2;
+}
 
 int launch_winmlp(const MlpFusedCall& c, hipStream_t stream) {
     if (!winmlp_supported(c.C, c.hidden) || c.M <= 0 || !c.x || !c.w1f || !c.w2f) {
@@ -500,7 +579,12 @@
     const WinMlpParams p = make_winmlp_params(c);
     const int nsplit = (c.C == 512 && c.slab && c.counters && c.nsplit == 2) ? 2 : 1;
     const double flops = 4.0 * c.M * (double)c.C * c.hidden;
-    const double bytes = 8.0 * c.M * (double)c.C + 4.0 * c.C * (double)c.hidden;
+    const bool exit_map = c.out_map.data != nullptr;
+    if (exit_map && !(winmlp_exit_supported(c) && c.out_ln_w && c.out_ln_b)) {
+        set_error("win_mlp: the stage-exit epilogue needs the 4-wave C = 256 form, no layer scale and both LayerNorm2d parameters (C=%d)", c.C);
+        return FVIT_EINVAL;
+    }
+    const double bytes = (exit_map ? 6.0 : 8.0) * c.M * (double)c.C + 4.0 * c.C * (double)c.hidden;
     ProfScope prof(FVIT_K_MLP_FUSED, flops, bytes, stream);
     const int form256 = c.C == 256 && !c.ts ? tune_get("win_mlp256", 2) : 2;
     const bool wide256 = form256 == 1;
@@ -538,7 +622,12 @@
         else hipLaunchKernelGGL((winmlp_kernel<_Float16, 256, 1024, 4, 2, 4, 1, 1, true>), dim3(grid), dim3(256), 0, stream, p);
     } else
 #endif
-    if (c.C == 512 && nsplit == 2) FVIT_WINMLP_ST(2);
+    if (exit_map) {
+#define FVIT_WINMLP_X(T, SP_) hipLaunchKernelGGL((winmlp_kernel<T, 256, 1024, 4, 2, 4, SP_, 1, false, false, true>), dim3(grid), dim3(256), 0, stream, p)
+        if (c.dtype == FVIT_F16) { if (c.terms == 2) FVIT_WINMLP_X(_Float16, 2); else FVIT_WINMLP_X(_Float16, 1); }
+        else { if (c.terms == 2) FVIT_WINMLP_X(__bf16, 2); else FVIT_WINMLP_X(__bf16, 1); }
+#undef FVIT_WINMLP_X
+    } else if (c.C == 512 && nsplit == 2) FVIT_WINMLP_ST(2);
     else if (c.C == 512 && pipe) FVIT_WINMLP_PT(512, 2048, 4, 8);
     else if (c.C == 512) FVIT_WINMLP_T(512, 2048, 4, 8);
     else if (wide256) FVIT_WINMLP_T(256, 1024, 8, 8);
```

New measurement: 93920 images/s, median of 6. +1.4%, better.
